# kai-neumann/OrthoSfM

Hardware: AMD Instinct MI355X
Metric: image-pairs matched/sec + BA iterations/sec (N images, M tracks) at 1/2/4/8 GPU (higher is better)
Workload: dtype i8; 1 GPU; 50 orthographic images, 20000 SIFT features/img, exhaustive matching (1225 pairs, low-res gate + two-way + cross-check + lists; SURVEY 8d's unit of work: up to, not including, RANSAC-F -- the pass through RANSAC-F is `with_geometric_verification`); views=50, features_per_view=20000, pairs=1225

## Files before the change

### orthosfm_amd/csrc/match_all.hip

```cpp
#include <algorithm>
#include <chrono>
#include <cstdlib>
#include <cstring>

#include "match_internal.h"
#include "ransac_kernels.h"
#include "ransac_affine.h"

namespace osfm {

namespace {

struct Lap {
    std::chrono::steady_clock::time_point t_chunk = std::chrono::steady_clock::now();
    void operator()(const char *what) const
    {
        static const bool trace = getenv("OSFM_MATCH_TRACE") != nullptr;
        if (trace) fprintf(stderr, "[osfm match] %-18s %9.3f ms\n", what,
            std::chrono::duration<double, std::milli>(std::chrono::steady_clock::now() - t_chunk).count());
    }
};

struct ChunkLists {
    std::vector<int64_t> m12_off, corr_off;
    std::vector<int32_t> len12;
    std::vector<uint8_t> keep;
};

int compact_chunk(osfm_matcher *m, const ChunkLists &h, int n, int64_t chunk_corr, int32_t *corr, int64_t written, int *chunk_no)
{
    const osfm_match_options &o = m->opts;
    hipStream_t s = m->stream;
    OSFM_RETURN_IF(m->d_m12_off.reserve(n * 8));
    OSFM_RETURN_IF(m->d_corr_off.reserve(n * 8));
    OSFM_RETURN_IF(m->d_len12.reserve(n * 4));
    OSFM_RETURN_IF(m->d_keep_pair.reserve(n));
    const int cb = o.geometric_verification ? 0 : ((*chunk_no)++ & 1);
    DeviceBuffer &dcorr = cb ? m->d_corr_alt : m->d_corr;
    if (m->copied_used[cb]) OSFM_HIP_CHECK(hipEventSynchronize(m->ev_copied[cb]));
    OSFM_RETURN_IF(dcorr.reserve((size_t)chunk_corr * 8));
    OSFM_HIP_CHECK(hipMemcpyAsync(m->d_m12_off.ptr, h.m12_off.data(), n * 8, hipMemcpyHostToDevice, s));
    OSFM_HIP_CHECK(hipMemcpyAsync(m->d_corr_off.ptr, h.corr_off.data(), n * 8, hipMemcpyHostToDevice, s));
    OSFM_HIP_CHECK(hipMemcpyAsync(m->d_len12.ptr, h.len12.data(), n * 4, hipMemcpyHostToDevice, s));
    OSFM_HIP_CHECK(hipMemcpyAsync(m->d_keep_pair.ptr, h.keep.data(), n, hipMemcpyHostToDevice, s));
    launch_compact_pairs(n, m->out.as<int32_t>(), m->d_m12_off.as<int64_t>(),
        m->d_len12.as<int32_t>(), m->d_corr_off.as<int64_t>(), m->d_keep_pair.as<uint8_t>(),
        dcorr.as<int32_t>(), s);
    OSFM_HIP_CHECK(hipGetLastError());
    if (!o.geometric_verification) {
        OSFM_HIP_CHECK(hipEventRecord(m->ev_compact[cb], s));
        OSFM_HIP_CHECK(hipStreamWaitEvent(m->copy_stream, m->ev_compact[cb], 0));
        OSFM_HIP_CHECK(hipMemcpyAsync(corr + 2 * written, dcorr.ptr, (size_t)chunk_corr * 8,
            hipMemcpyDeviceToHost, m->copy_stream));
        OSFM_HIP_CHECK(hipEventRecord(m->ev_copied[cb], m->copy_stream));
        m->copied_used[cb] = true;
    }
    return OSFM_OK;
}

int verify_chunk(osfm_matcher *m, const osfm_pair *pairs, const int *idx, int n, const std::vector<int32_t> &counts,
    const ChunkLists &h, int64_t chunk_corr, osfm_pair_result *results, int32_t *corr, int64_t capacity,
    int64_t *written_out, bool *overflow, const Lap &lap)
{
    const osfm_match_options &o = m->opts;
    hipStream_t s = m->stream;
    std::vector<RansacJob> jobs;
    std::vector<int> job_pair;
    OSFM_RETURN_IF(m->d_inl.reserve((size_t)chunk_corr * 4));
    OSFM_RETURN_IF(m->d_inl_count.reserve((size_t)n * 4));
    for (int k = 0; k < n; ++k) {
        if (!h.keep[k]) continue;
        const int p = idx[k];
        const ViewData &a = m->views[pairs[p].view_1], &b = m->views[pairs[p].view_2];
        if (a.n_positions < 0 || b.n_positions < 0) {
            set_error("match_all: geometric verification needs osfm_match_set_positions for views %d and %d",
                pairs[p].view_1, pairs[p].view_2);
            return OSFM_E_STATE;
        }
        RansacJob j;
        memset(&j, 0, sizeof(j));
        j.pos1 = a.positions.as<float>(); j.pos2 = b.positions.as<float>();
        j.corr = m->d_corr.as<int32_t>() + 2 * h.corr_off[k];
        j.k = counts[k];
        const int64_t hi = std::max(pairs[p].view_1, pairs[p].view_2), lo = std::min(pairs[p].view_1, pairs[p].view_2);
        j.pair_id = (uint64_t)(hi * (hi - 1) / 2 + lo);
        j.inliers_out = m->d_inl.as<int32_t>() + h.corr_off[k];
        j.count_out = m->d_inl_count.as<int32_t>() + (int)jobs.size();
        j.F_out = nullptr;
        jobs.push_back(j); job_pair.push_back(k);
    }
    const size_t jobs_bytes = (jobs.size() * sizeof(RansacJob) + 255) / 256 * 256;
    const bool affine = o.ransac_model == OSFM_RANSAC_AFFINE;
    OSFM_RETURN_IF(m->d_jobs.reserve(jobs_bytes + (affine ? affine_scratch_bytes((int)jobs.size()) : ransac_scratch_bytes((int)jobs.size()))));
    OSFM_HIP_CHECK(hipMemcpyAsync(m->d_jobs.ptr, jobs.data(), jobs.size() * sizeof(RansacJob), hipMemcpyHostToDevice, s));
    if (affine)
        launch_ransac_affine(m->d_jobs.as<RansacJob>(), (int)jobs.size(), o.ransac_max_iterations, o.ransac_threshold,
            o.ransac_refit, o.ransac_seed, static_cast<char *>(m->d_jobs.ptr) + jobs_bytes, nullptr, s);
    else
        launch_ransac(m->d_jobs.as<RansacJob>(), (int)jobs.size(), o.ransac_max_iterations, o.ransac_threshold,
            o.ransac_seed, static_cast<char *>(m->d_jobs.ptr) + jobs_bytes, s);
    OSFM_HIP_CHECK(hipGetLastError());
    std::vector<int32_t> h_cnt(jobs.size());
    OSFM_HIP_CHECK(hipMemcpyAsync(h_cnt.data(), m->d_inl_count.ptr, jobs.size() * 4, hipMemcpyDeviceToHost, s));
    lap("ransac queued");
    OSFM_HIP_CHECK(hipStreamSynchronize(s));
    lap("ransac done");
    const int min_inl = std::max(8, o.min_matching_inliers);
    std::vector<int64_t> g_src, g_dst;
    std::vector<int32_t> g_cnt;
    int64_t chunk_out = 0;
    for (size_t jx = 0; jx < jobs.size(); ++jx) {
        const int k = job_pair[jx];
        osfm_pair_result &r = results[idx[k]];
        r.num_inliers = h_cnt[jx];
        if (h_cnt[jx] < min_inl) { r.status = OSFM_PAIR_REJECTED_INLIERS; r.offset = 0; continue; }
        r.offset = *written_out + chunk_out;
        g_src.push_back(h.corr_off[k]); g_dst.push_back(chunk_out); g_cnt.push_back(h_cnt[jx]);
        chunk_out += h_cnt[jx];
    }
    if (*written_out + chunk_out > capacity) *overflow = true;
    if (!*overflow && chunk_out > 0) {
        const int ng = (int)g_cnt.size();
        OSFM_RETURN_IF(m->d_gather_off.reserve((size_t)ng * 20));
        OSFM_RETURN_IF(m->d_corr2.reserve((size_t)chunk_out * 8));
        char *gb = m->d_gather_off.as<char>();
        OSFM_HIP_CHECK(hipMemcpyAsync(gb, g_src.data(), (size_t)ng * 8, hipMemcpyHostToDevice, s));
        OSFM_HIP_CHECK(hipMemcpyAsync(gb + (size_t)ng * 8, g_dst.data(), (size_t)ng * 8, hipMemcpyHostToDevice, s));
        OSFM_HIP_CHECK(hipMemcpyAsync(gb + (size_t)ng * 16, g_cnt.data(), (size_t)ng * 4, hipMemcpyHostToDevice, s));
        launch_gather_inliers(ng, m->d_corr.as<int32_t>(), m->d_inl.as<int32_t>(),
            reinterpret_cast<const int64_t *>(gb), reinterpret_cast<const int64_t *>(gb + (size_t)ng * 8),
            reinterpret_cast<const int32_t *>(gb + (size_t)ng * 16), m->d_corr2.as<int32_t>(), s);
        OSFM_HIP_CHECK(hipGetLastError());
        OSFM_HIP_CHECK(hipMemcpyAsync(corr + 2 * *written_out, m->d_corr2.ptr, (size_t)chunk_out * 8,
            hipMemcpyDeviceToHost, s));
        OSFM_HIP_CHECK(hipStreamSynchronize(s));
        lap("lists on the host");
    }
    *written_out += chunk_out;
    return OSFM_OK;
}

}

int match_all_single(osfm_matcher *m, const osfm_pair *pairs, int num_pairs, osfm_pair_result *results,
    int32_t *corr, int64_t capacity, int64_t *total, int phase)
{
    std::lock_guard<std::mutex> lock(m->mu);
    OSFM_HIP_CHECK(hipSetDevice(m->device));
    if (phase != kPhaseFull) reset_stats(m);
    const osfm_match_options &o = m->opts;
    struct CopyDrain { hipStream_t s; ~CopyDrain() { if (s) (void)hipStreamSynchronize(s); } } copy_drain{m->copy_stream};

    std::vector<int> lowres_idx, full_idx;
    for (int p = 0; p < num_pairs; ++p) {
        OSFM_RETURN_IF(check_view(m, pairs[p].view_1, "match_all"));
        OSFM_RETURN_IF(check_view(m, pairs[p].view_2, "match_all"));
        const ViewData &a = m->views[pairs[p].view_1], &b = m->views[pairs[p].view_2];
        osfm_pair_result &r = results[p];
        if (phase == kPhaseFull) {
            if (r.status == OSFM_PAIR_MATCHED) full_idx.push_back(p);
            continue;
        }
        r.status = OSFM_PAIR_MATCHED; r.lowres_matches = -1; r.num_matches = 0; r.num_inliers = -1; r.offset = 0;
        const size_t np1 = (size_t)a.ns + a.nu, np2 = (size_t)b.ns + b.nu;
        if (np1 == 0 || np2 == 0) { r.status = OSFM_PAIR_SKIPPED_EMPTY; continue; }
        if (o.use_lowres_matching && np1 * np2 > 1000000) lowres_idx.push_back(p);
        else full_idx.push_back(p);
    }

    {
        const int bs = batch_size_for(m->views, o, true);
        std::vector<osfm_pair> chunk;
        for (size_t start = 0; start < lowres_idx.size(); start += bs) {
            const size_t end = std::min(lowres_idx.size(), start + bs);
            chunk.clear();
            for (size_t k = start; k < end; ++k) chunk.push_back(pairs[lowres_idx[k]]);
            BatchResult res;
            BatchMode mode;
            mode.limit = o.num_lowres_features; mode.lowres = true; mode.apply = false;
            OSFM_RETURN_IF(run_batch(m, chunk.data(), (int)chunk.size(), mode, &res));
            for (size_t k = start; k < end; ++k) {
                const int p = lowres_idx[k];
                results[p].lowres_matches = res.counts[k - start];
                if (res.counts[k - start] < o.min_lowres_matches)
                    results[p].status = OSFM_PAIR_REJECTED_LOWRES;
                else
                    full_idx.push_back(p);
            }
        }
        std::sort(full_idx.begin(), full_idx.end());
    }
    if (phase == kPhaseGate) { if (total) *total = 0; return OSFM_OK; }

    const int min_matches = std::max(8, o.min_feature_matches);
    int64_t written = 0, written_out = 0;
    bool overflow = false;
    {
        const int bs = full_batch_size(m->views, o, full_idx.size());
        int chunk_no = 0;
        std::vector<osfm_pair> chunk;
        ChunkLists h;
        for (size_t start = 0; start < full_idx.size(); start += bs) {
            const size_t end = std::min(full_idx.size(), start + bs);
            const int n = (int)(end - start);
            chunk.clear();
            for (size_t k = start; k < end; ++k) chunk.push_back(pairs[full_idx[k]]);
            const Lap lap{};
            BatchResult res;
            BatchMode full_mode;
            if (m->expect_pairs > 0)
                full_mode.expect = std::min<int>(full_batch_size(m->views, o, (size_t)m->expect_pairs), m->expect_pairs);
            OSFM_RETURN_IF(run_batch(m, chunk.data(), n, full_mode, &res));
            lap("matched");
            h.m12_off.assign(n, 0); h.corr_off.assign(n, 0); h.len12.assign(n, 0); h.keep.assign(n, 0);
            int64_t chunk_corr = 0;
            for (int k = 0; k < n; ++k) {
                const int p = full_idx[start + k];
                osfm_pair_result &r = results[p];
                r.num_matches = res.counts[k];
                if (res.counts[k] < min_matches) { r.status = OSFM_PAIR_REJECTED_COUNT; continue; }
                r.status = OSFM_PAIR_MATCHED;
                r.offset = written + chunk_corr;
                h.keep[k] = 1;
                h.m12_off[k] = res.plans[k].off12;
                h.len12[k] = res.plans[k].len12;
                h.corr_off[k] = chunk_corr;
                chunk_corr += res.counts[k];
            }
            if (!o.geometric_verification && written + chunk_corr > capacity) overflow = true;
            if (chunk_corr > 0 && (o.geometric_verification || !overflow))
                OSFM_RETURN_IF(compact_chunk(m, h, n, chunk_corr, corr, written, &chunk_no));
            if (o.geometric_verification && chunk_corr > 0)
                OSFM_RETURN_IF(verify_chunk(m, pairs, full_idx.data() + start, n, res.counts, h, chunk_corr, results, corr,
                    capacity, &written_out, &overflow, lap));
            written += chunk_corr;
        }
    }
    if (!o.geometric_verification) OSFM_HIP_CHECK(hipStreamSynchronize(m->copy_stream));
    if (o.geometric_verification) written = written_out;
    if (total) *total = written;
    if (overflow) {
        set_error("match_all: %lld correspondences need more than the given capacity %lld",
            (long long)written, (long long)capacity);
        return OSFM_E_CAPACITY;
    }
    return OSFM_OK;
}

}
```

### orthosfm_amd/csrc/match_api.hip

```cpp
#include <algorithm>
#include <cfloat>
#include <cmath>
#include <cstddef>
#include <cstring>

#include "match_internal.h"
#include "cashash_kernels.h"
#include "ransac_kernels.h"
#include "ransac_affine.h"
#include "view_front.h"

namespace osfm {

static thread_local std::string g_last_error;

void set_error(const char *fmt, ...)
{
    char buf[1024];
    va_list ap;
    va_start(ap, fmt);
    vsnprintf(buf, sizeof(buf), fmt, ap);
    va_end(ap);
    g_last_error = buf;
}

}

using namespace osfm;

extern "C" {

const char *osfm_last_error(void) { return g_last_error.c_str(); }
int osfm_version(void) { return OSFM_ABI_VERSION; }

int osfm_device_count(void)
{
    int n = 0;
    if (hipGetDeviceCount(&n) != hipSuccess) return 0;
    return n;
}

int osfm_ransac_selfcheck(int mode, uint64_t *counters)
{
    if (mode < 0 || mode > 2) { set_error("ransac_selfcheck: mode %d", mode); return OSFM_E_ARG; }
    int ndev = 0;
    if (hipGetDeviceCount(&ndev) != hipSuccess || ndev <= 0) {
        set_error("ransac_selfcheck: no HIP device available");
        return OSFM_E_DEVICE;
    }
    unsigned long long c[3] = {0, 0, 0};
    OSFM_RETURN_IF(ransac_set_mode(mode, c));
    if (counters) for (int i = 0; i < 3; ++i) counters[i] = c[i];
    return OSFM_OK;
}

int osfm_trim_device_memory(int device, uint64_t *released_bytes)
{
    int ndev = 0;
    if (hipGetDeviceCount(&ndev) != hipSuccess || ndev <= 0) {
        set_error("trim_device_memory: no HIP device available");
        return OSFM_E_DEVICE;
    }
    if (device < -1 || device >= ndev) { set_error("trim_device_memory: device %d out of range [-1,%d)", device, ndev); return OSFM_E_ARG; }
    const size_t b = g_device_pool.trim(device);
    if (released_bytes) *released_bytes = b;
    return OSFM_OK;
}

int osfm_device_memory(int device, uint64_t *free_bytes, uint64_t *total_bytes)
{
    int ndev = 0;
    if (hipGetDeviceCount(&ndev) != hipSuccess || ndev <= 0) {
        set_error("device_memory: no HIP device available");
        return OSFM_E_DEVICE;
    }
    if (device < 0 || device >= ndev) { set_error("device_memory: device %d out of range [0,%d)", device, ndev); return OSFM_E_ARG; }
    OSFM_HIP_CHECK(hipSetDevice(device));
    size_t f = 0, t = 0;
    OSFM_HIP_CHECK(hipMemGetInfo(&f, &t));
    if (free_bytes) *free_bytes = f;
    if (total_bytes) *total_bytes = t;
    return OSFM_OK;
}

int osfm_library_memory(osfm_memory_report *out)
{
    if (!out) { set_error("library_memory: null"); return OSFM_E_ARG; }
    out->device_buffer_bytes = g_ledger.device_buffer_bytes.load();
    out->pool_live_bytes = g_ledger.pool_live_bytes.load();
    out->pool_cached_bytes = g_ledger.pool_cached_bytes.load();
    out->pinned_host_bytes = g_ledger.pinned_host_bytes.load();
    out->live_matchers = g_ledger.live_matchers.load();
    out->live_streams = g_ledger.live_streams.load();
    out->live_events = g_ledger.live_events.load();
    out->reserved = 0;
    return OSFM_OK;
}

int osfm_match_options_default(osfm_match_options *o)
{
    if (!o) { set_error("options_default: null"); return OSFM_E_ARG; }
    o->sift_lowe_ratio = 0.8f;
    o->sift_distance_threshold = FLT_MAX;
    o->surf_lowe_ratio = 0.7f;
    o->surf_distance_threshold = FLT_MAX;
    o->use_lowres_matching = 1;
    o->num_lowres_features = 500;
    o->min_lowres_matches = 5;
    o->min_feature_matches = 50;
    o->pairs_per_batch = 0;
    o->geometric_verification = 0;
    o->ransac_max_iterations = 1000;
    o->ransac_threshold = 0.0015;
    o->min_matching_inliers = 30;
    o->matcher_type = OSFM_MATCHER_EXHAUSTIVE;
    o->ransac_seed = 0;
    o->cascade_keep_empty_blocks = 0;
    o->special_kernel_max = 0;
    o->ransac_model = OSFM_RANSAC_FUNDAMENTAL;
    o->ransac_refit = 1;
    return OSFM_OK;
}

int osfm_match_create(int device, int num_views, const osfm_match_options *opts, osfm_matcher **out)
{
    if (!out || num_views < 0) { set_error("match_create: bad arguments"); return OSFM_E_ARG; }
    *out = nullptr;
    if (opts && opts->ransac_model != OSFM_RANSAC_FUNDAMENTAL && opts->ransac_model != OSFM_RANSAC_AFFINE) {
        set_error("match_create: ransac_model %d", opts->ransac_model);
        return OSFM_E_ARG;
    }
    int ndev = 0;
    if (hipGetDeviceCount(&ndev) != hipSuccess || ndev <= 0) {
        set_error("match_create: no HIP device available (this backend has no CPU fallback)");
        return OSFM_E_DEVICE;
    }
    if (device < 0 || device >= ndev) {
        set_error("match_create: device %d out of range [0,%d)", device, ndev);
        return OSFM_E_ARG;
    }
    OSFM_HIP_CHECK(hipSetDevice(device));
    struct Owner { osfm_matcher *p; ~Owner() { if (p) osfm_match_destroy(p); } } owner{(g_ledger.live_matchers++, new osfm_matcher())};
    osfm_matcher *m = owner.p;
    m->device = device;
    if (opts) m->opts = *opts; else osfm_match_options_default(&m->opts);
    m->views = std::vector<ViewData>(num_views);
    reset_stats(m);
    OSFM_HIP_CHECK(stream_create(&m->stream));
    for (int i = 0; i < 2; ++i)
        for (int j = 0; j < 2; ++j) OSFM_HIP_CHECK(event_create(&m->ev[i][j], true));
    for (int j = 0; j < 2; ++j) OSFM_HIP_CHECK(event_create(&m->ev_sp[j], true));
    for (int j = 0; j < 2; ++j) OSFM_HIP_CHECK(event_create(&m->pin_ev[j], false));
    OSFM_HIP_CHECK(stream_create(&m->copy_stream));
    OSFM_HIP_CHECK(stream_create(&m->up_stream));
    for (int j = 0; j < 2; ++j) {
        OSFM_HIP_CHECK(event_create(&m->ev_compact[j], false));
        OSFM_HIP_CHECK(event_create(&m->ev_copied[j], false));
    }
    if (m->opts.special_kernel_max != 0) m->special_max = std::min(std::max(m->opts.special_kernel_max, 0), 512);
    std::vector<int32_t> t;
    build_lowe_table(m->opts.sift_lowe_ratio, false, &t);
    OSFM_RETURN_IF(m->lowe_sift.reserve(t.size() * 4));
    OSFM_HIP_CHECK(hipMemcpy(m->lowe_sift.ptr, t.data(), t.size() * 4, hipMemcpyHostToDevice));
    build_lowe_table(m->opts.surf_lowe_ratio, true, &t);
    OSFM_RETURN_IF(m->lowe_surf.reserve(t.size() * 4));
    OSFM_HIP_CHECK(hipMemcpy(m->lowe_surf.ptr, t.data(), t.size() * 4, hipMemcpyHostToDevice));
    m->tab_sift.reject_from = m->lowe_sift.as<int32_t>();
    m->tab_sift.max_d1 = max_d1_for(m->opts.sift_distance_threshold, false);
    m->tab_sift.is_signed = 0;
    m->tab_surf.reject_from = m->lowe_surf.as<int32_t>();
    m->tab_surf.max_d1 = max_d1_for(m->opts.surf_distance_threshold, true);
    m->tab_surf.is_signed = 1;
    owner.p = nullptr;
    *out = m;
    return OSFM_OK;
}

int osfm_match_create_multi(const int *device_ids, int num_devices, int num_views,
    const osfm_match_options *opts, osfm_matcher **out)
{
    if (!out || !device_ids || num_devices < 1 || num_views < 0) { set_error("match_create_multi: bad arguments"); return OSFM_E_ARG; }
    *out = nullptr;
    if (opts && opts->ransac_model != OSFM_RANSAC_FUNDAMENTAL && opts->ransac_model != OSFM_RANSAC_AFFINE) {
        set_error("match_create_multi: ransac_model %d", opts->ransac_model);
        return OSFM_E_ARG;
    }
    struct Owner { osfm_matcher *p; ~Owner() { if (p) osfm_match_destroy(p); } } owner{(g_ledger.live_matchers++, new osfm_matcher())};
    osfm_matcher *m = owner.p;
    m->device = device_ids[0];
    if (opts) m->opts = *opts; else osfm_match_options_default(&m->opts);
    reset_stats(m);
    for (int k = 0; k < num_devices; ++k) {
        osfm_matcher *sh = nullptr;
        OSFM_RETURN_IF(osfm_match_create(device_ids[k], num_views, &m->opts, &sh));
        m->shards.push_back(sh);
    }
    m->shard_stage.resize(num_devices);
    owner.p = nullptr;
    *out = m;
    return OSFM_OK;
}

int osfm_match_get_devices(const osfm_matcher *m, int32_t *device_ids, int capacity, int32_t *num_devices)
{
    if (!m || !num_devices || capacity < 0 || (capacity > 0 && !device_ids)) { set_error("match_get_devices: bad arguments"); return OSFM_E_ARG; }
    const int n = m->shards.empty() ? 1 : (int)m->shards.size();
    *num_devices = n;
    for (int k = 0; k < std::min(n, capacity); ++k) device_ids[k] = m->shards.empty() ? m->device : m->shards[k]->device;
    return OSFM_OK;
}

int osfm_match_destroy(osfm_matcher *m)
{
    if (!m) return OSFM_OK;
    if (!m->shards.empty() || !m->shard_stage.empty()) {
        for (auto *sh : m->shards) osfm_match_destroy(sh);
        for (auto &sg : m->shard_stage) pinned_free(sg.ptr, sg.ints * 4);
        g_ledger.live_matchers--;
        delete m;
        return OSFM_OK;
    }
    (void)hipSetDevice(m->device);
    if (m->stream) (void)hipStreamSynchronize(m->stream);
    for (int i = 0; i < 2; ++i)
        for (int j = 0; j < 2; ++j) event_destroy(m->ev[i][j]);
    for (int j = 0; j < 2; ++j) event_destroy(m->ev_sp[j]);
    for (int j = 0; j < 2; ++j) {
        event_destroy(m->pin_ev[j]);
        pinned_free(m->pin_ptr[j], m->pin_bytes[j]);
    }
    stream_destroy(m->copy_stream);
    stream_destroy(m->up_stream);
    for (int j = 0; j < 2; ++j) {
        event_destroy(m->ev_compact[j]);
        event_destroy(m->ev_copied[j]);
    }
    stream_destroy(m->stream);
    for (auto *sg : m->comb_staging) { pinned_free(sg->ptr, sg->ints * 4); delete sg; }
    g_ledger.live_matchers--;
    delete m;
    return OSFM_OK;
}

int osfm_quantize_sift(const float *src, int n, uint16_t *dst)
{
    if (n < 0 || (n > 0 && (!src || !dst))) { set_error("quantize_sift: bad arguments"); return OSFM_E_ARG; }
    for (size_t i = 0; i < (size_t)n * 128; ++i) {
        float v = src[i];
        v = v < 0.0f ? 0.0f : (v > 1.0f ? 1.0f : v);
        v *= 255.0f;
        v = v > 0.0f ? floorf(v + 0.5f) : ceilf(v - 0.5f);
        dst[i] = (uint16_t)(unsigned char)v;
    }
    return OSFM_OK;
}

int osfm_quantize_surf(const float *src, int n, int16_t *dst)
{
    if (n < 0 || (n > 0 && (!src || !dst))) { set_error("quantize_surf: bad arguments"); return OSFM_E_ARG; }
    for (size_t i = 0; i < (size_t)n * 64; ++i) {
        float v = src[i];
        v = v < -1.0f ? -1.0f : (v > 1.0f ? 1.0f : v);
        v *= 127.0f;
        v = v > 0.0f ? floorf(v + 0.5f) : ceilf(v - 0.5f);
        dst[i] = (int16_t)(signed char)v;
    }
    return OSFM_OK;
}

int osfm_match_set_view(osfm_matcher *m, int view, const uint16_t *sift, int n_sift,
    const int16_t *surf, int n_surf)
{
    if (!m) { set_error("set_view: null matcher"); return OSFM_E_ARG; }
    if (!m->shards.empty())
        return for_each_shard(m, [&](size_t k) { return osfm_match_set_view(m->shards[k], view, sift, n_sift, surf, n_surf); });
    std::lock_guard<std::mutex> lock(m->up_mu);
    OSFM_HIP_CHECK(hipSetDevice(m->device));
    return upload_view(m, view, sift, n_sift, surf, n_surf);
}

int osfm_match_set_view_float(osfm_matcher *m, int view, const float *sift, int n_sift,
    const float *surf, int n_surf)
{
    if (!m) { set_error("set_view_float: null matcher"); return OSFM_E_ARG; }
    if (n_sift < 0 || n_surf < 0) { set_error("set_view_float: negative count"); return OSFM_E_ARG; }
    std::vector<uint16_t> qs((size_t)n_sift * 128);
    std::vector<int16_t> qu((size_t)n_surf * 64);
    OSFM_RETURN_IF(osfm_quantize_sift(sift, n_sift, qs.data()));
    OSFM_RETURN_IF(osfm_quantize_surf(surf, n_surf, qu.data()));
    return osfm_match_set_view(m, view, qs.data(), n_sift, qu.data(), n_surf);
}

int osfm_match_expect_pairs(osfm_matcher *m, int32_t pairs_per_call)
{
    if (!m || pairs_per_call < 0) { set_error("match_expect_pairs: bad arguments"); return OSFM_E_ARG; }
    if (!m->shards.empty()) {
        for (auto *sh : m->shards) sh->expect_pairs = (pairs_per_call + (int)m->shards.size() - 1) / (int)m->shards.size();
        return OSFM_OK;
    }
    std::lock_guard<std::mutex> lock(m->mu);
    m->expect_pairs = pairs_per_call;
    return OSFM_OK;
}

int osfm_match_view_size(const osfm_matcher *m, int view, int *n_sift, int *n_surf)
{
    if (!m) { set_error("view_size: null matcher"); return OSFM_E_ARG; }
    if (!m->shards.empty()) return osfm_match_view_size(m->shards[0], view, n_sift, n_surf);
    OSFM_RETURN_IF(check_view(m, view, "view_size"));
    if (n_sift) *n_sift = m->views[view].ns;
    if (n_surf) *n_surf = m->views[view].nu;
    return OSFM_OK;
}

int osfm_match_set_positions(osfm_matcher *m, int view, const float *xy, int n)
{
    if (!m || n < 0 || (n > 0 && !xy)) { set_error("set_positions: bad argument"); return OSFM_E_ARG; }
    if (!m->shards.empty())
        return for_each_shard(m, [&](size_t k) { return osfm_match_set_positions(m->shards[k], view, xy, n); });
    std::lock_guard<std::mutex> lock(m->mu);
    OSFM_HIP_CHECK(hipSetDevice(m->device));
    OSFM_RETURN_IF(check_view(m, view, "set_positions"));
    ViewData &v = m->views[view];
    if (n != v.ns + v.nu) {
        set_error("set_positions: view %d has %d features, got %d positions", view, v.ns + v.nu, n);
        return OSFM_E_ARG;
    }
    OSFM_RETURN_IF(v.positions.reserve((size_t)std::max(n, 1) * 8));
    if (n) OSFM_HIP_CHECK(hipMemcpy(v.positions.ptr, xy, (size_t)n * 8, hipMemcpyHostToDevice));
    v.n_positions = n;
    return OSFM_OK;
}

int osfm_match_set_view_from_front(osfm_matcher *m, int view, osfm_view_front *front)
{
    if (!m || !front) { set_error("set_view_from_front: null argument"); return OSFM_E_ARG; }
    FrontResult r;
    OSFM_RETURN_IF(view_front_result(front, &r));
    return handoff_all(m, view, r.device, r.sift_desc, r.sift_map, r.n_sift, r.surf_desc, r.surf_map, r.n_surf, r.normalized,
        [&](hipStream_t s) { return view_front_begin_read(front, s); }, [&](hipStream_t s) { return view_front_end_read(front, s); });
}

int osfm_match_debug_set_view_device(osfm_matcher *m, int view, const float *sift, int n_sift, const int32_t *sift_order,
    const float *surf, int n_surf, const int32_t *surf_order, const float *positions)
{
    if (!m || n_sift < 0 || n_surf < 0 || (n_sift > 0 && !sift) || (n_surf > 0 && !surf) || (n_sift + n_surf > 0 && !positions)) {
        set_error("debug_set_view_device: bad arguments");
        return OSFM_E_ARG;
    }
    for (int i = 0; i < n_sift; ++i)
        if (sift_order && (sift_order[i] < 0 || sift_order[i] >= n_sift)) { set_error("debug_set_view_device: sift_order[%d] out of range", i); return OSFM_E_ARG; }
    for (int i = 0; i < n_surf; ++i)
        if (surf_order && (surf_order[i] < 0 || surf_order[i] >= n_surf)) { set_error("debug_set_view_device: surf_order[%d] out of range", i); return OSFM_E_ARG; }
    const int device = m->shards.empty() ? m->device : m->shards[0]->device;
    OSFM_HIP_CHECK(hipSetDevice(device));
    DeviceBuffer d_sift, d_surf, d_so, d_uo, d_pos;
    auto put = [](DeviceBuffer &b, const void *src, size_t bytes) -> int {
        if (!src || !bytes) return OSFM_OK;
        OSFM_RETURN_IF(b.reserve(bytes));
        OSFM_HIP_CHECK(hipMemcpy(b.ptr, src, bytes, hipMemcpyHostToDevice));
        return OSFM_OK;
    };
    OSFM_RETURN_IF(put(d_sift, sift, (size_t)n_sift * 128 * 4));
    OSFM_RETURN_IF(put(d_surf, surf, (size_t)n_surf * 64 * 4));
    OSFM_RETURN_IF(put(d_so, sift_order, (size_t)n_sift * 4));
    OSFM_RETURN_IF(put(d_uo, surf_order, (size_t)n_surf * 4));
    OSFM_RETURN_IF(put(d_pos, positions, (size_t)(n_sift + n_surf) * 8));
    hipStream_t used = nullptr;
    const int rc = handoff_all(m, view, device, d_sift.as<float>(), d_so.as<int32_t>(), n_sift, d_surf.as<float>(), d_uo.as<int32_t>(),
        n_surf, d_pos.as<float>(), [&](hipStream_t s) -> int { used = s; return OSFM_OK; }, [](hipStream_t) -> int { return OSFM_OK; });
    if (used) (void)hipStreamSynchronize(used);
    return rc;
}

int osfm_match_debug_view_bank(osfm_matcher *m, int view, int shard, osfm_view_bank *b)
{
    if (!m || !b) { set_error("debug_view_bank: null argument"); return OSFM_E_ARG; }
    if (!m->shards.empty()) {
        if (shard < 0 || shard >= (int)m->shards.size()) { set_error("debug_view_bank: shard %d of %zu", shard, m->shards.size()); return OSFM_E_ARG; }
        return osfm_match_debug_view_bank(m->shards[(size_t)shard], view, 0, b);
    }
    std::lock_guard<std::mutex> lock(m->up_mu);
    OSFM_HIP_CHECK(hipSetDevice(m->device));
    OSFM_RETURN_IF(check_view(m, view, "debug_view_bank"));
    const ViewData &v = m->views[view];
    OSFM_HIP_CHECK(hipStreamSynchronize(m->up_stream));
    const int sp_pad = v.n_special > 0 ? round_up(v.n_special, kRowsPerBlock) : 0;
    b->n_sift = v.ns; b->n_surf = v.nu; b->n_sift_pad = v.ns_pad; b->n_surf_pad = v.nu_pad;
    b->n_special = v.n_special; b->n_special_pad = sp_pad; b->surf_norm2_max = v.surf_norm2_max; b->n_positions = v.n_positions;
    struct { void *to; const DeviceBuffer *from; size_t bytes; } arrays[] = {
        {b->sift, &v.sift, (size_t)v.ns_pad * 128}, {b->sift_corr, &v.sift_corr, (size_t)v.ns_pad * 4},
        {b->sift_raw, &v.sift_raw, (size_t)v.ns_pad * 128}, {b->sift_raw_corr, &v.sift_raw_corr, (size_t)v.ns_pad * 4},
        {b->surf, &v.surf, (size_t)v.nu_pad * 64}, {b->surf_corr, &v.surf_corr, (size_t)v.nu_pad * 4},
        {b->special, &v.special, (size_t)sp_pad * 128}, {b->special_corr, &v.special_corr, (size_t)sp_pad * 4},
        {b->special_map, &v.special_map, sp_pad ? (size_t)v.n_special * 4 : 0},
        {b->special_slot, &v.special_slot, sp_pad ? (size_t)v.ns * 4 : 0},
        {b->positions, &v.positions, (size_t)std::max(v.n_positions, 0) * 8},
    };
    for (auto &r : arrays)
        if (r.to && r.bytes) OSFM_HIP_CHECK(hipMemcpy(r.to, r.from->ptr, r.bytes, hipMemcpyDeviceToHost));
    return OSFM_OK;
}

int osfm_ransac_options_default(osfm_ransac_options *o)
{
    if (!o) { set_error("ransac_options_default: null"); return OSFM_E_ARG; }
    o->max_iterations = 1000; o->reserved = 0; o->threshold = 0.0015; o->seed = 0;
    return OSFM_OK;
}

}

template <class Launch>
static int ransac_single_pair(const char *name, int min_k, size_t scratch_bytes, int device, const float *pos1, int n1,
    const float *pos2, int n2, const int32_t *corr, int k, uint64_t pair_id, int32_t *inliers, int32_t *num_inliers,
    double *F, void *result, size_t result_bytes, Launch launch)
{
    if (n1 < 0 || n2 < 0 || k < 0 || !num_inliers || (k > 0 && (!pos1 || !pos2 || !corr || !inliers))) {
        set_error("%s: bad argument", name); return OSFM_E_ARG;
    }
    for (int i = 0; i < k; ++i)
        if (corr[2 * i] < 0 || corr[2 * i] >= n1 || corr[2 * i + 1] < 0 || corr[2 * i + 1] >= n2) {
            set_error("%s: correspondence %d out of range", name, i); return OSFM_E_ARG;
        }
    int ndev = 0;
    if (hipGetDeviceCount(&ndev) != hipSuccess || ndev <= 0) {
        set_error("%s: no HIP device available (this backend has no CPU fallback)", name);
        return OSFM_E_DEVICE;
    }
    if (device < 0 || device >= ndev) { set_error("%s: bad device", name); return OSFM_E_ARG; }
    OSFM_HIP_CHECK(hipSetDevice(device));
    if (k < min_k) { *num_inliers = -1; return OSFM_OK; }
    DeviceBuffer d1, d2, dc, di, dn, df, dj, dr;
    struct Rel { DeviceBuffer *b[8]; ~Rel() { for (auto *x : b) x->release(); } } rel{{&d1, &d2, &dc, &di, &dn, &df, &dj, &dr}};
    OSFM_RETURN_IF(d1.reserve((size_t)n1 * 8)); OSFM_RETURN_IF(d2.reserve((size_t)n2 * 8));
    OSFM_RETURN_IF(dc.reserve((size_t)k * 8)); OSFM_RETURN_IF(di.reserve((size_t)k * 4));
    OSFM_RETURN_IF(dn.reserve(16)); OSFM_RETURN_IF(df.reserve(72));
    if (result_bytes) OSFM_RETURN_IF(dr.reserve(result_bytes));
    OSFM_RETURN_IF(dj.reserve(256 + scratch_bytes));
    OSFM_HIP_CHECK(hipMemcpy(d1.ptr, pos1, (size_t)n1 * 8, hipMemcpyHostToDevice));
    OSFM_HIP_CHECK(hipMemcpy(d2.ptr, pos2, (size_t)n2 * 8, hipMemcpyHostToDevice));
    OSFM_HIP_CHECK(hipMemcpy(dc.ptr, corr, (size_t)k * 8, hipMemcpyHostToDevice));
    RansacJob job;
    memset(&job, 0, sizeof(job));
    job.pos1 = d1.as<float>(); job.pos2 = d2.as<float>(); job.corr = dc.as<int32_t>(); job.k = k;
    job.pair_id = pair_id; job.inliers_out = di.as<int32_t>(); job.count_out = dn.as<int32_t>();
    job.F_out = df.as<double>();
    OSFM_HIP_CHECK(hipMemcpy(dj.ptr, &job, sizeof(job), hipMemcpyHostToDevice));
    launch(dj.as<RansacJob>(), static_cast<char *>(dj.ptr) + 256, dr.ptr);
    OSFM_HIP_CHECK(hipGetLastError());
    OSFM_HIP_CHECK(hipDeviceSynchronize());
    int32_t cnt = 0;
    OSFM_HIP_CHECK(hipMemcpy(&cnt, dn.ptr, 4, hipMemcpyDeviceToHost));
    *num_inliers = cnt;
    if (cnt > 0) OSFM_HIP_CHECK(hipMemcpy(inliers, di.ptr, (size_t)cnt * 4, hipMemcpyDeviceToHost));
    if (F) OSFM_HIP_CHECK(hipMemcpy(F, df.ptr, 72, hipMemcpyDeviceToHost));
    if (result) OSFM_HIP_CHECK(hipMemcpy(result, dr.ptr, result_bytes, hipMemcpyDeviceToHost));
    return OSFM_OK;
}

extern "C" {

int osfm_ransac_fundamental(int device, const float *pos1, int n1, const float *pos2, int n2,
    const int32_t *corr, int k, const osfm_ransac_options *opts, uint64_t pair_id,
    int32_t *inliers, int32_t *num_inliers, double *F)
{
    osfm_ransac_options o;
    if (opts) o = *opts; else osfm_ransac_options_default(&o);
    return ransac_single_pair("ransac_fundamental", 8, ransac_scratch_bytes(1), device, pos1, n1, pos2, n2, corr, k, pair_id,
        inliers, num_inliers, F, nullptr, 0, [&](const RansacJob *d_job, void *scratch, void *) {
            launch_ransac(d_job, 1, o.max_iterations, o.threshold, o.seed, scratch, nullptr);
        });
}

int osfm_ransac_affine_options_default(osfm_ransac_affine_options *o)
{
    if (!o) { set_error("ransac_affine_options_default: null"); return OSFM_E_ARG; }
    o->max_iterations = 1000; o->refit = 1; o->threshold = 0.0015; o->seed = 0;
    return OSFM_OK;
}

int osfm_ransac_affine(int device, const float *pos1, int n1, const float *pos2, int n2,
    const int32_t *corr, int k, const osfm_ransac_affine_options *opts, uint64_t pair_id,
    int32_t *inliers, int32_t *num_inliers, double *F, osfm_ransac_affine_result *result)
{
    osfm_ransac_affine_options o;
    if (opts) o = *opts; else osfm_ransac_affine_options_default(&o);
    return ransac_single_pair("ransac_affine", 4, affine_scratch_bytes(1), device, pos1, n1, pos2, n2, corr, k, pair_id,
        inliers, num_inliers, F, result, sizeof(*result), [&](const RansacJob *d_job, void *scratch, void *d_result) {
            launch_ransac_affine(d_job, 1, o.max_iterations, o.threshold, o.refit, o.seed, scratch,
                static_cast<osfm_ransac_affine_result *>(d_result), nullptr);
        });
}

int osfm_match_pair(osfm_matcher *m, int view_1, int view_2, int32_t *m12, int32_t *len12,
    int32_t *m21, int32_t *len21)
{
    if (!m || !m12 || !m21) { set_error("match_pair: null argument"); return OSFM_E_ARG; }
    if (!m->shards.empty())
        return osfm_match_pair(m->shards[m->next_shard++ % m->shards.size()], view_1, view_2, m12, len12, m21, len21);
    OSFM_RETURN_IF(check_view(m, view_1, "match"));
    OSFM_RETURN_IF(check_view(m, view_2, "match"));
    osfm_matcher::PairRequest rq;
    rq.kind = 0; rq.v1 = view_1; rq.v2 = view_2; rq.num_features = 0;
    rq.m12 = m12; rq.m21 = m21; rq.len12 = len12; rq.len21 = len21; rq.count = nullptr;
    return combine(m, rq);
}

int osfm_match_pair_lowres(osfm_matcher *m, int view_1, int view_2, int num_features, int32_t *count)
{
    if (!m || !count) { set_error("match_pair_lowres: null argument"); return OSFM_E_ARG; }
    if (!m->shards.empty())
        return osfm_match_pair_lowres(m->shards[m->next_shard++ % m->shards.size()], view_1, view_2, num_features, count);
    if (num_features <= 0) { *count = 0; return OSFM_OK; }
    OSFM_RETURN_IF(check_view(m, view_1, "match"));
    OSFM_RETURN_IF(check_view(m, view_2, "match"));
    osfm_matcher::PairRequest rq;
    rq.kind = 1; rq.v1 = view_1; rq.v2 = view_2; rq.num_features = num_features;
    rq.m12 = rq.m21 = rq.len12 = rq.len21 = nullptr; rq.count = count;
    return combine(m, rq);
}

int osfm_match_twoway(osfm_matcher *m, int view_1, int view_2, int descriptor_type, int num_features,
    int32_t *m12, int32_t *m21)
{
    if (!m || !m12 || !m21 || (descriptor_type != 0 && descriptor_type != 1) || num_features < 0) {
        set_error("match_twoway: bad argument");
        return OSFM_E_ARG;
    }
    if (!m->shards.empty()) return osfm_match_twoway(m->shards[0], view_1, view_2, descriptor_type, num_features, m12, m21);
    std::lock_guard<std::mutex> lock(m->mu);
    OSFM_HIP_CHECK(hipSetDevice(m->device));
    reset_stats(m);
    osfm_pair pr = {view_1, view_2};
    BatchResult res;
    BatchMode mode;
    mode.limit = num_features; mode.apply = false; mode.type_mask = 1 << descriptor_type;
    OSFM_RETURN_IF(run_batch(m, &pr, 1, mode, &res));
    const PairPlan &pl = res.plans[0];
    const ViewData &a = m->views[view_1], &b = m->views[view_2];
    int n1 = descriptor_type == 0 ? a.ns : a.nu, n2 = descriptor_type == 0 ? b.ns : b.nu;
    if (num_features > 0) { n1 = std::min(n1, num_features); n2 = std::min(n2, num_features); }
    if (n1 == 0) { for (int i = 0; i < n2; ++i) m21[i] = -1; return OSFM_OK; }
    const int32_t *d_out = m->out.as<int32_t>();
    if (pl.len12) OSFM_HIP_CHECK(hipMemcpy(m12, d_out + pl.off12, (size_t)pl.len12 * 4, hipMemcpyDeviceToHost));
    if (pl.len21) OSFM_HIP_CHECK(hipMemcpy(m21, d_out + pl.off21, (size_t)pl.len21 * 4, hipMemcpyDeviceToHost));
    return OSFM_OK;
}

int osfm_pair_from_index(int64_t index, int32_t *view_1, int32_t *view_2)
{
    if (index < 0 || !view_1 || !view_2) { set_error("pair_from_index: bad arguments"); return OSFM_E_ARG; }
    const int a = (int)(0.5 + std::sqrt(0.25 + 2.0 * (double)index));
    *view_1 = a;
    *view_2 = (int)index - a * (a - 1) / 2;
    return OSFM_OK;
}

int osfm_match_all(osfm_matcher *m, const osfm_pair *pairs, int num_pairs, osfm_pair_result *results,
    int32_t *corr, int64_t capacity, int64_t *total)
{
    if (!m || (num_pairs > 0 && (!pairs || !results)) || num_pairs < 0 || capacity < 0 ||
        (capacity > 0 && !corr)) {
        set_error("match_all: bad arguments");
        return OSFM_E_ARG;
    }
    if (!m->shards.empty()) return multi_match_all(m, pairs, num_pairs, results, corr, capacity, total);
    return match_all_single(m, pairs, num_pairs, results, corr, capacity, total, kPhaseBoth);
}

int osfm_match_get_cascade_hashes(osfm_matcher *m, int view, int type, uint64_t *hashes,
    uint8_t *bucket_ids)
{
    if (!m || type < 0 || type > 1) { set_error("get_cascade_hashes: bad arguments"); return OSFM_E_ARG; }
    if (!m->shards.empty()) return osfm_match_get_cascade_hashes(m->shards[0], view, type, hashes, bucket_ids);
    std::lock_guard<std::mutex> lock(m->mu);
    OSFM_RETURN_IF(check_view(m, view, "get_cascade_hashes"));
    OSFM_HIP_CHECK(hipSetDevice(m->device));
    OSFM_RETURN_IF(ensure_cashash(m));
    const ViewData &v = m->views[view];
    const int n = type == 0 ? v.ns : v.nu;
    const int words = type == 0 ? 2 : 1;
    if (n > 0 && hashes)
        OSFM_HIP_CHECK(hipMemcpy(hashes, v.cas_hash[type].ptr, (size_t)n * words * 8, hipMemcpyDeviceToHost));
    if (n > 0 && bucket_ids)
        OSFM_HIP_CHECK(hipMemcpy(bucket_ids, v.cas_bucket[type].ptr, (size_t)n * kCasGroups, hipMemcpyDeviceToHost));
    return OSFM_OK;
}

int osfm_match_get_shard_stats(const osfm_matcher *m, int shard, osfm_match_stats *out)
{
    if (!m || !out) { set_error("get_shard_stats: null argument"); return OSFM_E_ARG; }
    const int n = m->shards.empty() ? 1 : (int)m->shards.size();
    if (shard < 0 || shard >= n) { set_error("get_shard_stats: shard %d of %d", shard, n); return OSFM_E_ARG; }
    *out = m->shards.empty() ? m->stats : m->shards[shard]->stats;
    return OSFM_OK;
}

int osfm_match_get_stats(const osfm_matcher *m, osfm_match_stats *out)
{
    if (!m || !out) { set_error("get_stats: null argument"); return OSFM_E_ARG; }
    if (!m->shards.empty()) {
        memset(out, 0, sizeof(*out));
        for (const auto *sh : m->shards) {
            const osfm_match_stats &t = sh->stats;
            out->tile_kernel_ms += t.tile_kernel_ms; out->tile_kernel_launches += t.tile_kernel_launches;
            out->exact_scan_queries += t.exact_scan_queries; out->mac_count += t.mac_count;
            out->algorithmic_bytes += t.algorithmic_bytes; out->lowres_kernel_ms += t.lowres_kernel_ms;
            out->lowres_kernel_launches += t.lowres_kernel_launches; out->lowres_mac_count += t.lowres_mac_count;
            out->cashash_kernel_ms += t.cashash_kernel_ms; out->cashash_kernel_launches += t.cashash_kernel_launches;
            out->special_kernel_launches += t.special_kernel_launches; out->special_kernel_ms += t.special_kernel_ms;
            out->tile_shader_cycles += t.tile_shader_cycles; out->tile_refclk_ticks += t.tile_refclk_ticks;
            out->surf_tile_kernel_ms += t.surf_tile_kernel_ms; out->surf_tile_kernel_launches += t.surf_tile_kernel_launches;
            out->surf_mac_count += t.surf_mac_count; out->tile_workgroups += t.tile_workgroups;
        }
        return OSFM_OK;
    }
    *out = m->stats;
    return OSFM_OK;
}

#undef osfm_match_options_default
#undef osfm_match_create
#undef osfm_match_create_multi
static constexpr size_t kOptionsBytesBefore = offsetof(osfm_match_options, ransac_model);
static_assert(kOptionsBytesBefore == 80, "the layout binaries built against the earlier header pass");

static osfm_match_options options_from_before(const void *opts)
{
    osfm_match_options o;
    memset(&o, 0, sizeof(o));
    osfm_match_options_default_v2(&o);
    if (opts) memcpy(&o, opts, kOptionsBytesBefore);
    return o;
}

OSFM_API int osfm_match_options_default(void *opts)
{
    if (!opts) { set_error("options_default: null"); return OSFM_E_ARG; }
    const osfm_match_options o = options_from_before(nullptr);
    memcpy(opts, &o, kOptionsBytesBefore);
    return OSFM_OK;
}

OSFM_API int osfm_match_create(int device, int num_views, const void *opts, osfm_matcher **out)
{
    const osfm_match_options o = options_from_before(opts);
    return osfm_match_create_v2(device, num_views, &o, out);
}

OSFM_API int osfm_match_create_multi(const int *device_ids, int num_devices, int num_views, const void *opts, osfm_matcher **out)
{
    const osfm_match_options o = options_from_before(opts);
    return osfm_match_create_multi_v2(device_ids, num_devices, num_views, &o, out);
}

}
```

### orthosfm_amd/csrc/match_batch.hip

```cpp
#include <algorithm>
#include <cstdlib>
#include <cstring>

#include "match_internal.h"
#include "cashash_kernels.h"

namespace osfm {

int check_view(const osfm_matcher *m, int v, const char *what) { return check_view(m->views, v, what); }

void reset_stats(osfm_matcher *m) { memset(&m->stats, 0, sizeof(m->stats)); }

int run_batch(osfm_matcher *m, const osfm_pair *pairs, int num_pairs, const BatchMode &mode,
    BatchResult *res)
{
    const bool cascade = cascade_batch(m->opts, mode);
    if (cascade) OSFM_RETURN_IF(ensure_cashash(m));
    static const int forced_seg_tiles = [] { const char *e = getenv("OSFM_SEG_TILES"); return e ? atoi(e) : 0; }();
    const char *rescan_env = getenv("OSFM_FINISH_RESCAN");
    PlanKnobs knobs;
    knobs.seg_tiles = forced_seg_tiles;
    knobs.rescan_wave = rescan_env && strcmp(rescan_env, "wave") == 0;
    BatchPlan &plan = m->plan;
    res->counts.assign(num_pairs, 0);
    OSFM_RETURN_IF(plan_batch(m->views, m->opts, m->special_max, knobs, pairs, num_pairs, mode, &plan));
    res->plans = plan.plans;
    res->out_ints = plan.out_ints;
    const std::vector<PairPlan> &plans = plan.plans;
    std::vector<MatchProblem> *probs = plan.probs;
    const std::vector<SpecialJob> &spjobs = plan.spjobs, &spjobs_wide = plan.spjobs_wide;
    const int64_t out_ints = plan.out_ints, total_queries = plan.total_queries, rs_buckets = plan.rs_buckets;
    const int *total_blocks = plan.total_blocks, *max_n = plan.max_n;

    double grow = 1.0;
    if (mode.expect > num_pairs && num_pairs > 0) grow = 1.02 * (double)mode.expect / num_pairs;
    auto grown = [&](int64_t n) { return (size_t)((double)std::max<int64_t>(n, 1) * std::max(grow, 1.0)); };
    OSFM_RETURN_IF(m->out.reserve(grown(std::max<int64_t>(out_ints, 4)) * 4));
    OSFM_RETURN_IF(m->rowparts.reserve(grown(plan.rowpart_recs) * sizeof(RowPart)));
    OSFM_RETURN_IF(m->colparts.reserve(grown(plan.colpart_recs) * sizeof(ColPart)));
    OSFM_RETURN_IF(m->keep.reserve(grown(std::max<int64_t>(plan.keep_bytes, 16))));
    OSFM_RETURN_IF(m->exact_items.reserve(grown(total_queries) * sizeof(ExactItem)));
    OSFM_RETURN_IF(m->exact_count.reserve(16));
    if (plan.bucketed) {
        OSFM_RETURN_IF(m->rs_count.reserve(grown(rs_buckets) * sizeof(int32_t)));
        OSFM_RETURN_IF(m->rs_items.reserve(grown(plan.rs_items) * sizeof(RescoreItem)));
    }
    OSFM_RETURN_IF(m->sp_parts.reserve((size_t)std::max<int64_t>(plan.sp_recs, 1) * sizeof(RowPart)));
    hipStream_t s = m->stream;
    {
        std::vector<uint8_t> seen(m->views.size(), 0);
        for (int p = 0; p < num_pairs; ++p)
            for (int v : {plans[p].v1, plans[p].v2})
                if (!seen[v]) { seen[v] = 1; if (m->views[v].ready) OSFM_HIP_CHECK(hipStreamWaitEvent(s, m->views[v].ready, 0)); }
    }
    OSFM_RETURN_IF(m->sp_col.reserve((size_t)std::max<int64_t>(plan.sp_cols, 1) * 4));
    OSFM_RETURN_IF(m->d_spjobs.reserve(std::max<size_t>(spjobs.size() + spjobs_wide.size(), 1) * sizeof(SpecialJob)));
    if (!spjobs.empty())
        OSFM_HIP_CHECK(hipMemcpyAsync(m->d_spjobs.ptr, spjobs.data(), spjobs.size() * sizeof(SpecialJob),
            hipMemcpyHostToDevice, s));
    if (!spjobs_wide.empty())
        OSFM_HIP_CHECK(hipMemcpyAsync(m->d_spjobs.as<SpecialJob>() + spjobs.size(), spjobs_wide.data(),
            spjobs_wide.size() * sizeof(SpecialJob), hipMemcpyHostToDevice, s));
    int32_t *d_out = m->out.as<int32_t>();
    OSFM_HIP_CHECK(hipMemsetAsync(d_out, 0xff, (size_t)std::max<int64_t>(out_ints, 4) * 4, s));

    OSFM_HIP_CHECK(hipMemsetAsync(m->exact_count.ptr, 0, 16, s));
    bool timed[2] = {false, false};
    bool probed = false;
    for (int type = 0; type < 2; ++type) {
        const int np = (int)probs[type].size();
        if (np == 0) continue;
        for (int i = 0; i < np; ++i) {
            probs[type][i].m12 = d_out + plan.m12_off[type][i];
            probs[type][i].m21 = d_out + plan.m21_off[type][i];
        }
        OSFM_RETURN_IF(m->d_problems[type].reserve(np * sizeof(MatchProblem)));
        OSFM_RETURN_IF(m->mark_off[type].reserve(np * 2 * sizeof(int64_t)));
        OSFM_RETURN_IF(m->counts[type].reserve(np * sizeof(int32_t)));
        OSFM_HIP_CHECK(hipMemcpyAsync(m->d_problems[type].ptr, probs[type].data(),
            np * sizeof(MatchProblem), hipMemcpyHostToDevice, s));
        OSFM_HIP_CHECK(hipMemcpyAsync(m->mark_off[type].ptr, plan.mark_off[type].data(),
            np * 2 * sizeof(int64_t), hipMemcpyHostToDevice, s));
        OSFM_HIP_CHECK(hipMemsetAsync(m->counts[type].ptr, 0, np * sizeof(int32_t), s));
        const MatchProblem *dp = m->d_problems[type].as<MatchProblem>();
        const LoweTable tab = type == 0 ? m->tab_sift : m->tab_surf;
        const int ecap = (int)std::min<int64_t>(total_queries, 0x7fffffff);
        int32_t *ecount = m->exact_count.as<int32_t>() + type;

        if (cascade) {
            OSFM_HIP_CHECK(hipEventRecord(m->ev[type][0], s));
            timed[type] = true;
            OSFM_RETURN_IF(m->cas_state.reserve((size_t)std::max<int64_t>(plan.cas_queries[type], 1) * kCasMaxCand * 4));
            launch_cashash_match(type == 0 ? 128 : 64, dp, np, max_n[type], m->cas_state.as<int32_t>(), tab, s);
            OSFM_HIP_CHECK(hipEventRecord(m->ev[type][1], s));
        } else {
            if (total_blocks[type] > 0) { OSFM_HIP_CHECK(hipEventRecord(m->ev[type][0], s)); timed[type] = true; }
            unsigned long long *probe = nullptr;
            if (type == 0 && mode.limit == 0) {
                OSFM_RETURN_IF(m->clock_probe.reserve(16));
                OSFM_HIP_CHECK(hipMemsetAsync(m->clock_probe.ptr, 0, 16, s));
                probe = m->clock_probe.as<unsigned long long>();
                probed = true;
            }
            if (!m->zero_tile.ptr) {
                OSFM_RETURN_IF(m->zero_tile.reserve((size_t)kTileCols * 128));
                OSFM_HIP_CHECK(hipMemsetAsync(m->zero_tile.ptr, 0, (size_t)kTileCols * 128, s));
            }
            launch_match_tiles(type == 0 ? 8 : 4, plan.needs_mask[type], plan.any_special[type], plan.any_c0[type],
                plan.any_corrected[type], dp, np, total_blocks[type],
                m->rowparts.as<RowPart>(), m->colparts.as<ColPart>(), s, probe, m->zero_tile.as<int8_t>());
            if (timed[type]) OSFM_HIP_CHECK(hipEventRecord(m->ev[type][1], s));
            if (type == 0 && !(spjobs.empty() && spjobs_wide.empty())) {
                OSFM_HIP_CHECK(hipEventRecord(m->ev_sp[0], s));
                launch_match_special(dp, m->d_spjobs.as<SpecialJob>(), (int)spjobs.size(), m->sp_parts.as<RowPart>(),
                    m->sp_col.as<int32_t>(), s);
                launch_match_special_wide(dp, m->d_spjobs.as<SpecialJob>() + spjobs.size(), (int)spjobs_wide.size(),
                    m->sp_parts.as<RowPart>(), m->sp_col.as<int32_t>(), s);
                OSFM_HIP_CHECK(hipEventRecord(m->ev_sp[1], s));
            }
            const bool rs = type == 0 && plan.bucketed;
            if (rs) OSFM_HIP_CHECK(hipMemsetAsync(m->rs_count.ptr, 0, (size_t)rs_buckets * sizeof(int32_t), s));
            launch_match_finish(dp, np, max_n[type], m->rowparts.as<RowPart>(),
                m->colparts.as<ColPart>(), m->sp_parts.as<RowPart>(), m->sp_col.as<int32_t>(), tab, 0,
                m->exact_items.as<ExactItem>(), ecount, ecap, rs ? m->rs_count.as<int32_t>() : nullptr,
                rs ? m->rs_items.as<RescoreItem>() : nullptr, s);
            if (rs)
                launch_match_rescore(dp, np, m->rs_count.as<int32_t>(), m->rs_items.as<RescoreItem>(), rs_buckets, tab,
                    m->exact_items.as<ExactItem>(), ecount, ecap, s);
            launch_exact_scan(type == 0 ? 128 : 64, dp, m->exact_items.as<ExactItem>(), ecount, ecap,
                tab, s);
        }
        launch_cross_check_mark(dp, np, max_n[type], m->keep.as<uint8_t>(), m->keep.as<uint8_t>(),
            m->mark_off[type].as<int64_t>(), m->counts[type].as<int32_t>(), s);
        if (mode.apply)
            launch_cross_check_apply(dp, np, max_n[type], m->keep.as<uint8_t>(),
                m->keep.as<uint8_t>(), m->mark_off[type].as<int64_t>(), s);
        OSFM_HIP_CHECK(hipGetLastError());
    }

    std::vector<int32_t> hc[2];
    int32_t hexact[4] = {0, 0, 0, 0};
    for (int type = 0; type < 2; ++type) {
        hc[type].resize(probs[type].size());
        if (!hc[type].empty())
            OSFM_HIP_CHECK(hipMemcpyAsync(hc[type].data(), m->counts[type].ptr,
                hc[type].size() * sizeof(int32_t), hipMemcpyDeviceToHost, s));
    }
    OSFM_HIP_CHECK(hipMemcpyAsync(hexact, m->exact_count.ptr, 16, hipMemcpyDeviceToHost, s));
    unsigned long long hprobe[2] = {0, 0};
    if (probed) OSFM_HIP_CHECK(hipMemcpyAsync(hprobe, m->clock_probe.ptr, 16, hipMemcpyDeviceToHost, s));
    OSFM_HIP_CHECK(hipStreamSynchronize(s));
    m->stats.tile_shader_cycles += (double)hprobe[0];
    m->stats.tile_refclk_ticks += (double)hprobe[1];
    for (int p = 0; p < num_pairs; ++p) {
        int c = 0;
        for (int type = 0; type < 2; ++type)
            if (plans[p].prob_index[type] >= 0) c += hc[type][plans[p].prob_index[type]];
        res->counts[p] = c;
    }
    for (int type = 0; type < 2; ++type) {
        if (!timed[type]) continue;
        float ms = 0.f;
        OSFM_HIP_CHECK(hipEventElapsedTime(&ms, m->ev[type][0], m->ev[type][1]));
        if (cascade) {
            m->stats.cashash_kernel_ms += ms;
            m->stats.cashash_kernel_launches += 1;
        } else if (mode.limit > 0) {
            m->stats.lowres_kernel_ms += ms;
            m->stats.lowres_kernel_launches += 1;
        } else {
            m->stats.tile_kernel_ms += ms;
            m->stats.tile_kernel_launches += 1;
            m->stats.tile_workgroups += total_blocks[type];
            if (type == 1) { m->stats.surf_tile_kernel_ms += ms; m->stats.surf_tile_kernel_launches += 1; }
        }
    }
    if (!(spjobs.empty() && spjobs_wide.empty())) {
        float ms = 0.f;
        OSFM_HIP_CHECK(hipEventElapsedTime(&ms, m->ev_sp[0], m->ev_sp[1]));
        m->stats.special_kernel_ms += ms;
        m->stats.special_kernel_launches += 1;
    }
    m->stats.exact_scan_queries += hexact[0] + hexact[1];
    if (cascade) {
    } else if (mode.limit > 0) {
        m->stats.lowres_mac_count += plan.macs;
    } else {
        m->stats.mac_count += plan.macs;
        m->stats.surf_mac_count += plan.macs_surf;
        m->stats.algorithmic_bytes += plan.alg_bytes;
    }
    return OSFM_OK;
}

}
```

### orthosfm_amd/csrc/match_internal.h

```cpp
#pragma once
#include <atomic>
#include <condition_variable>
#include <deque>
#include <functional>
#include <mutex>
#include <string>
#include <vector>

#include "match_plan.h"

struct osfm_matcher {
    int device = 0;
    hipStream_t stream = nullptr;
    osfm_match_options opts;
    std::vector<osfm::ViewData> views;
    osfm::DeviceBuffer lowe_sift, lowe_surf;
    osfm::LoweTable tab_sift, tab_surf;
    std::mutex mu;
    hipStream_t up_stream = nullptr;
    std::mutex up_mu;

    osfm::DeviceBuffer d_problems[2], rowparts, colparts, out, keep, mark_off[2], counts[2];
    osfm::DeviceBuffer exact_items, exact_count, stage_in, flags;
    osfm::DeviceBuffer rs_count, rs_items;
    osfm::DeviceBuffer sp_parts, sp_col, d_spjobs;
    osfm::DeviceBuffer clock_probe;
    osfm::BatchPlan plan;
    osfm::DeviceBuffer zero_tile;
    int special_max = 512;
    int expect_pairs = 0;
    osfm::DeviceBuffer d_m12_off, d_len12, d_corr_off, d_keep_pair, d_corr;
    osfm::DeviceBuffer d_corr_alt;
    hipStream_t copy_stream = nullptr;
    hipEvent_t ev_compact[2] = {nullptr, nullptr}, ev_copied[2] = {nullptr, nullptr};
    bool copied_used[2] = {false, false};
    osfm::DeviceBuffer d_jobs, d_inl, d_inl_count, d_corr2, d_gather_off;
    hipEvent_t ev[2][2] = {{nullptr, nullptr}, {nullptr, nullptr}};
    hipEvent_t ev_sp[2] = {nullptr, nullptr};
    char *pin_ptr[2] = {nullptr, nullptr};
    size_t pin_bytes[2] = {0, 0};
    hipEvent_t pin_ev[2] = {nullptr, nullptr};
    bool pin_used[2] = {false, false};
    unsigned pin_next = 0;

    osfm::DeviceBuffer cas_proj[2], cas_sum[2], cas_avg[2], cas_state;
    std::atomic<bool> cas_dirty{true};

    osfm_match_stats stats;

    struct Staging { int32_t *ptr = nullptr; size_t ints = 0; int users = 0; };
    struct PairRequest {
        int kind;
        int v1, v2, num_features;
        int32_t *m12, *m21, *len12, *len21, *count;
        int status = OSFM_OK;
        bool done = false;
        std::string error;
        Staging *stage = nullptr;
        int64_t src12 = 0, src21 = 0;
        int32_t n12 = 0, n21 = 0;
    };
    std::vector<Staging *> comb_staging;

    std::vector<osfm_matcher *> shards;
    std::vector<Staging> shard_stage;
    std::atomic<unsigned> next_shard{0};
    std::mutex multi_mu;
    std::mutex comb_mu;
    std::condition_variable comb_cv;
    std::deque<PairRequest *> comb_queue;
    bool comb_leader = false;
};

namespace osfm {

int check_view(const osfm_matcher *m, int v, const char *what);
int run_batch(osfm_matcher *m, const osfm_pair *pairs, int num_pairs, const BatchMode &mode, BatchResult *res);
void reset_stats(osfm_matcher *m);

int upload_view(osfm_matcher *m, int view, const uint16_t *sift, int n_sift, const int16_t *surf, int n_surf);
int handoff_all(osfm_matcher *m, int view, int device, const float *d_sift, const int32_t *sift_map, int n_sift,
    const float *d_surf, const int32_t *surf_map, int n_surf, const float *d_positions,
    const std::function<int(hipStream_t)> &begin, const std::function<int(hipStream_t)> &end);
int ensure_cashash(osfm_matcher *m);

enum { kPhaseBoth = 0, kPhaseGate = 1, kPhaseFull = 2 };
int match_all_single(osfm_matcher *m, const osfm_pair *pairs, int num_pairs, osfm_pair_result *results,
    int32_t *corr, int64_t capacity, int64_t *total, int phase);

int for_each_shard(osfm_matcher *m, const std::function<int(size_t)> &fn);
int multi_match_all(osfm_matcher *m, const osfm_pair *pairs, int num_pairs, osfm_pair_result *results,
    int32_t *corr, int64_t capacity, int64_t *total);

int combine(osfm_matcher *m, osfm_matcher::PairRequest &rq);

}
```

### orthosfm_amd/csrc/match_plan.h

```cpp
#pragma once
#include <cstdint>
#include <vector>

#include "match_kernels.h"
#include "osfm_common.h"

namespace osfm {

inline int round_up(int x, int m) { return (x + m - 1) / m * m; }

struct ViewData {
    bool set = false;
    int ns = 0, nu = 0;
    int ns_pad = 0, nu_pad = 0;
    DeviceBuffer sift, sift_corr, surf, surf_corr;
    DeviceBuffer sift_raw, sift_raw_corr, special, special_corr, special_map, special_slot;
    int n_special = 0;
    int surf_norm2_max = 0;
    DeviceBuffer cas_hash[2], cas_bucket[2], cas_start[2], cas_items[2], cas_rec[2];
    DeviceBuffer positions;
    int n_positions = -1;
    hipEvent_t ready = nullptr;
    ~ViewData() { event_destroy(ready); }
    ViewData() = default;
    ViewData(const ViewData &) = delete;
    ViewData &operator=(const ViewData &) = delete;
};

struct PairPlan {
    int v1, v2;
    int ns1, nu1, ns2, nu2;
    bool has_sift, has_surf;
    int64_t off12, off21;
    int len12, len21;
    int prob_index[2];
};

struct BatchResult {
    std::vector<PairPlan> plans;
    std::vector<int32_t> counts;
    int64_t out_ints = 0;
};

struct BatchMode {
    int limit = 0;
    bool lowres = false;
    bool apply = true;
    int type_mask = 3;
    int expect = 0;
};

inline bool cascade_batch(const osfm_match_options &opts, const BatchMode &mode)
{
    return opts.matcher_type == OSFM_MATCHER_CASCADE_HASHING && mode.limit == 0;
}

struct PlanKnobs {
    int seg_tiles = 0;
    bool rescan_wave = false;
};

struct BatchPlan {
    std::vector<PairPlan> plans;
    std::vector<MatchProblem> probs[2];
    std::vector<int64_t> m12_off[2], m21_off[2];
    std::vector<int64_t> mark_off[2];
    std::vector<SpecialJob> spjobs, spjobs_wide;
    int64_t out_ints = 0, rowpart_recs = 0, colpart_recs = 0, keep_bytes = 0, total_queries = 0;
    int64_t sp_recs = 0, sp_cols = 0;
    int64_t rs_buckets = 0, rs_items = 0;
    int64_t cas_queries[2] = {0, 0};
    int total_blocks[2] = {0, 0}, max_n[2] = {0, 0};
    bool needs_mask[2] = {false, false};
    bool any_special[2] = {false, false};
    bool any_c0[2] = {false, false}, any_corrected[2] = {false, false};
    bool bucketed = false, cascade = false;
    int64_t macs = 0, macs_surf = 0, alg_bytes = 0;
    void clear();
};

int check_view(const std::vector<ViewData> &views, int v, const char *what);

int plan_batch(const std::vector<ViewData> &views, const osfm_match_options &opts, int special_max, const PlanKnobs &knobs,
    const osfm_pair *pairs, int num_pairs, const BatchMode &mode, BatchPlan *out);

int batch_size_for(const std::vector<ViewData> &views, const osfm_match_options &o, bool lowres);
int full_batch_size(const std::vector<ViewData> &views, const osfm_match_options &o, size_t n_full);

void deal_pairs_lpt(const std::vector<ViewData> &views, int num_shards, const osfm_pair *pairs, const std::vector<int> &cand,
    std::vector<std::vector<int>> *owner);

void build_lowe_table(float lowe, bool is_signed, std::vector<int32_t> *tab);
int max_d1_for(float dist_thres, bool is_signed);

}
```

### orthosfm_amd/csrc/match_plan.hip

```cpp
#include <algorithm>
#include <climits>
#include <cstring>
#include <queue>

#include "match_plan.h"

namespace osfm {

int check_view(const std::vector<ViewData> &views, int v, const char *what)
{
    if (v < 0 || v >= (int)views.size()) {
        set_error("%s: view id %d out of range [0, %zu)", what, v, views.size());
        return OSFM_E_ARG;
    }
    if (!views[v].set) {
        set_error("%s: view %d has not been set", what, v);
        return OSFM_E_STATE;
    }
    return OSFM_OK;
}

void BatchPlan::clear()
{
    BatchPlan fresh;
    auto keep = [](auto &to, auto &from) { from.clear(); to.swap(from); };
    keep(fresh.plans, plans);
    keep(fresh.spjobs, spjobs);
    keep(fresh.spjobs_wide, spjobs_wide);
    for (int type = 0; type < 2; ++type) {
        keep(fresh.probs[type], probs[type]);
        keep(fresh.m12_off[type], m12_off[type]);
        keep(fresh.m21_off[type], m21_off[type]);
        keep(fresh.mark_off[type], mark_off[type]);
    }
    *this = std::move(fresh);
}

int plan_batch(const std::vector<ViewData> &views, const osfm_match_options &opts, int special_max, const PlanKnobs &knobs,
    const osfm_pair *pairs, int num_pairs, const BatchMode &mode, BatchPlan *out)
{
    BatchPlan &bp = *out;
    bp.clear();
    const int lowres_limit = mode.limit;
    const bool cascade = bp.cascade = cascade_batch(opts, mode);
    bp.plans.assign(num_pairs, PairPlan());
    struct SpEntry { int problem, side, view, units, nchunk; };
    std::vector<SpEntry> spentries;

    int64_t rb_estimate = 0;
    for (int p = 0; p < num_pairs; ++p) {
        const int v1 = pairs[p].view_1;
        if (v1 >= 0 && v1 < (int)views.size())
            rb_estimate += (std::max(views[v1].ns, views[v1].nu) + kRowsPerBlock - 1) / kRowsPerBlock;
    }
    auto choose_seg_cols = [&](int n2) {
        const int ncyc = (n2 + kCycleCols - 1) / kCycleCols;
        int cyc;
        if (knobs.seg_tiles > 0) cyc = std::max(1, knobs.seg_tiles / 16);
        else {
            constexpr int64_t kWantBlocks = 2048;
            const int64_t want = (kWantBlocks + std::max<int64_t>(rb_estimate, 1) - 1) / std::max<int64_t>(rb_estimate, 1);
            const int nseg = (int)std::min<int64_t>(std::max<int64_t>(want, 1), ncyc);
            cyc = (ncyc + nseg - 1) / nseg;
        }
        cyc = std::min(cyc, kSegColsMax / kCycleCols);
        return cyc * kCycleCols;
    };

    for (int p = 0; p < num_pairs; ++p) {
        PairPlan &pl = bp.plans[p];
        pl.v1 = pairs[p].view_1; pl.v2 = pairs[p].view_2;
        OSFM_RETURN_IF(check_view(views, pl.v1, "match"));
        OSFM_RETURN_IF(check_view(views, pl.v2, "match"));
        const ViewData &a = views[pl.v1], &b = views[pl.v2];
        pl.ns1 = a.ns; pl.nu1 = a.nu; pl.ns2 = b.ns; pl.nu2 = b.nu;
        pl.has_sift = a.ns > 0 && (mode.type_mask & 1);
        pl.has_surf = a.nu > 0 && (mode.type_mask & 2);
        if (cascade && !opts.cascade_keep_empty_blocks) {
            if (b.ns == 0) pl.has_sift = false;
            if (b.nu == 0) pl.has_surf = false;
        }
        if (mode.lowres && pl.has_sift) pl.has_surf = false;
        if (lowres_limit > 0) {
            pl.ns1 = std::min(pl.ns1, lowres_limit); pl.ns2 = std::min(pl.ns2, lowres_limit);
            pl.nu1 = std::min(pl.nu1, lowres_limit); pl.nu2 = std::min(pl.nu2, lowres_limit);
        }
        const int e1 = pl.has_sift ? pl.ns1 : 0;
        const int e2 = pl.has_sift ? pl.ns2 : 0;
        pl.len12 = e1 + (pl.has_surf ? pl.nu1 : 0);
        pl.len21 = e2 + (pl.has_surf ? pl.nu2 : 0);
        pl.off12 = bp.out_ints; bp.out_ints += round_up(pl.len12, 4);
        pl.off21 = bp.out_ints; bp.out_ints += round_up(pl.len21, 4);
        pl.prob_index[0] = pl.prob_index[1] = -1;
        for (int type = 0; type < 2; ++type) {
            if (type == 0 ? !pl.has_sift : !pl.has_surf) continue;
            MatchProblem pr;
            memset(&pr, 0, sizeof(pr));
            pr.n1 = type == 0 ? pl.ns1 : pl.nu1;
            pr.n2 = type == 0 ? pl.ns2 : pl.nu2;
            pr.A = (type == 0 ? a.sift : a.surf).as<int8_t>();
            pr.B = (type == 0 ? b.sift : b.surf).as<int8_t>();
            pr.corrA = (type == 0 ? a.sift_corr : a.surf_corr).as<int32_t>();
            pr.corrB = (type == 0 ? b.sift_corr : b.surf_corr).as<int32_t>();
            pr.A_raw = (type == 0 ? a.sift_raw : a.surf).as<int8_t>();
            pr.corrA_raw = (type == 0 ? a.sift_raw_corr : a.surf_corr).as<int32_t>();
            const bool limited = lowres_limit > 0;
            const int n_special = (type == 0 && !limited) ? a.n_special : 0;
            pr.n_special = n_special;
            pr.A_special = a.special.as<int8_t>();
            pr.corrA_special = a.special_corr.as<int32_t>();
            pr.special_map = a.special_map.as<int32_t>();
            pr.special_slot = n_special > 0 ? a.special_slot.as<int32_t>() : nullptr;
            const bool empty = pr.n1 == 0 || pr.n2 == 0;
            if (limited) bp.needs_mask[type] = true;
            pr.B_raw = (type == 0 ? b.sift_raw : b.surf).as<int8_t>();
            pr.c0 = (type == 1 || b.n_special == 0) ? 1 : 0;
            if (type == 0 && !limited && !cascade && !empty && (a.n_special > 0 || b.n_special > 0) &&
                a.n_special <= special_max && b.n_special <= special_max) {
                pr.sp = 1; pr.c0 = 1;
                pr.nsA = a.n_special; pr.nsB = b.n_special;
                pr.n_special = 0;
                pr.special_slot = a.n_special > 0 ? a.special_slot.as<int32_t>() : nullptr;
                pr.B_special = b.special.as<int8_t>();
                pr.corrB_special = b.special_corr.as<int32_t>();
                pr.special_map_B = b.special_map.as<int32_t>();
                pr.special_slot_B = b.n_special > 0 ? b.special_slot.as<int32_t>() : nullptr;
                for (int side = 0; side < 2; ++side) {
                    const int ns = side == 0 ? pr.nsA : pr.nsB, no = side == 0 ? pr.n2 : pr.n1;
                    if (ns == 0) continue;
                    const int units = (ns + 31) / 32;
                    pr.sp_wide[side] = units > kSpSlots ? 1 : 0;
                    const int chunk_cols = pr.sp_wide[side] ? kSpWideChunk : kSpChunk;
                    const int nchunk = (no + chunk_cols - 1) / chunk_cols;
                    pr.sp_row_off[side] = bp.sp_recs; bp.sp_recs += (int64_t)nchunk * round_up(ns, 32);
                    pr.sp_col_off[side] = bp.sp_cols; bp.sp_cols += round_up(no, 32);
                    spentries.push_back({(int)bp.probs[type].size(), side, side == 0 ? pl.v2 : pl.v1, units, nchunk});
                }
            }
            if (!empty && !limited) (pr.c0 ? bp.any_c0 : bp.any_corrected)[type] = true;
            if (!empty && pr.n_special > 0) bp.any_special[type] = true;
            pr.nrb_main = empty ? 0 : (pr.n1 + kRowsPerBlock - 1) / kRowsPerBlock;
            pr.nrb = pr.nrb_main + (empty ? 0 : (pr.n_special + kRowsPerBlock - 1) / kRowsPerBlock);
            pr.seg_cols = (pr.c0 && !limited && pr.n_special == 0 && !empty) ? choose_seg_cols(pr.n2) : kSegCols;
            pr.nseg = empty ? 0 : (pr.n2 + pr.seg_cols - 1) / pr.seg_cols;
            pr.n2stride = round_up(pr.n2, kCycleCols);
            pr.block_start = bp.total_blocks[type];
            pr.rs_bucket_off = bp.rs_buckets;
            pr.rs_item_off = bp.rs_items;
            if (type == 0 && !cascade && !empty) {
                bp.rs_buckets += rescore_buckets(pr.nrb_main, pr.n2);
                bp.rs_items += rescore_items(pr.nrb_main, pr.n2);
            }
            if (cascade) {
                const ViewData *vd[2] = {&a, &b};
                for (int side = 0; side < 2; ++side) {
                    pr.cas_rec[side] = vd[side]->cas_rec[type].ptr;
                    pr.cas_start[side] = vd[side]->cas_start[type].as<int32_t>();
                    pr.cas_items[side] = vd[side]->cas_items[type].as<int32_t>();
                }
                pr.cas_state_off[0] = bp.cas_queries[type]; bp.cas_queries[type] += pr.n1;
                pr.cas_state_off[1] = bp.cas_queries[type]; bp.cas_queries[type] += pr.n2;
            } else {
                bp.total_blocks[type] += pr.nrb * pr.nseg;
                pr.rowpart_off = bp.rowpart_recs;
                bp.rowpart_recs += (int64_t)pr.nseg * pr.nrb * kRowsPerBlock;
                pr.colpart_off = bp.colpart_recs;
                bp.colpart_recs += (int64_t)pr.nrb * pr.n2stride;
            }
            bp.m12_off[type].push_back(pl.off12 + (type == 0 ? 0 : e1));
            bp.m21_off[type].push_back(pl.off21 + (type == 0 ? 0 : e2));
            pr.out_off12 = (type == 1 && mode.apply) ? e2 : 0;
            pr.out_off21 = (type == 1 && mode.apply) ? e1 : 0;
            if (type == 1) {
                const long long bound = (long long)a.surf_norm2_max * (long long)b.surf_norm2_max;
                pr.force_exact = bound > 32767LL * 32767LL ? 1 : 0;
            }
            pl.prob_index[type] = (int)bp.probs[type].size();
            bp.mark_off[type].push_back(bp.keep_bytes); bp.keep_bytes += round_up(pr.n1, 16);
            bp.mark_off[type].push_back(bp.keep_bytes); bp.keep_bytes += round_up(pr.n2, 16);
            bp.max_n[type] = std::max(bp.max_n[type], std::max(pr.n1, pr.n2));
            bp.total_queries += pr.n1 + pr.n2;
            bp.probs[type].push_back(pr);
            if (!empty) {
                const int dim = type == 0 ? 128 : 64;
                bp.macs += (int64_t)pr.n1 * pr.n2 * dim;
                if (type == 1) bp.macs_surf += (int64_t)pr.n1 * pr.n2 * dim;
                bp.alg_bytes += (int64_t)(pr.n1 + pr.n2) * (dim + 4);
            }
        }
    }
    bp.bucketed = bp.rs_buckets > 0 && bp.rs_buckets <= INT_MAX && bp.max_n[0] < (1 << 26) && !knobs.rescan_wave;

    std::stable_sort(spentries.begin(), spentries.end(), [](const SpEntry &x, const SpEntry &y) {
        return x.view != y.view ? x.view < y.view : x.units < y.units;
    });
    for (size_t e = 0; e < spentries.size();) {
        SpecialJob j;
        memset(&j, 0, sizeof(j));
        const SpEntry &f = spentries[e];
        if (f.units > kSpSlots) {
            j.problem[0] = f.problem; j.side[0] = f.side; j.count = 0;
            for (int c = 0; c < f.nchunk; ++c) { j.chunk = c; bp.spjobs_wide.push_back(j); }
            ++e;
            continue;
        }
        if (f.units > 1) {
            j.problem[0] = f.problem; j.side[0] = f.side; j.count = 0;
            ++e;
        } else {
            int c = 0;
            while (c < kSpSlots && e < spentries.size() && spentries[e].view == f.view && spentries[e].units == 1) {
                j.problem[c] = spentries[e].problem; j.side[c] = spentries[e].side; ++c; ++e;
            }
            j.count = c;
        }
        for (int c = 0; c < f.nchunk; ++c) { j.chunk = c; bp.spjobs.push_back(j); }
    }
    return OSFM_OK;
}

int batch_size_for(const std::vector<ViewData> &views, const osfm_match_options &o, bool lowres)
{
    if (o.pairs_per_batch > 0) return o.pairs_per_batch;
    if (lowres) return 16384;
    size_t worst = 1;
    for (const auto &v : views) {
        const size_t n = (size_t)std::max(v.ns, v.nu) + 256;
        worst = std::max(worst, (n / kRowsPerBlock + 1) * n * sizeof(ColPart) + n * 64);
    }
    const size_t budget = (size_t)24 << 30;
    return (int)std::max<size_t>(1, std::min<size_t>(budget / worst, 4096));
}

int full_batch_size(const std::vector<ViewData> &views, const osfm_match_options &o, size_t n_full)
{
    int bs = batch_size_for(views, o, false);
    if (o.pairs_per_batch <= 0 && !o.geometric_verification && o.matcher_type != OSFM_MATCHER_CASCADE_HASHING && n_full >= 768)
        bs = std::min<int>(bs, (int)((n_full + 2) / 3));
    if (o.pairs_per_batch <= 0 && n_full > (size_t)bs) {
        const size_t parts = (n_full + bs - 1) / bs;
        bs = (int)((n_full + parts - 1) / parts);
    }
    return bs;
}

void deal_pairs_lpt(const std::vector<ViewData> &views, int num_shards, const osfm_pair *pairs, const std::vector<int> &cand,
    std::vector<std::vector<int>> *owner)
{
    const int n = num_shards;
    owner->assign(n, {});
    const int nc = (int)cand.size();
    std::vector<int64_t> w(nc);
    bool uniform = true;
    for (int i = 0; i < nc; ++i) {
        const ViewData &a = views[pairs[cand[i]].view_1], &b = views[pairs[cand[i]].view_2];
        w[i] = (int64_t)(a.ns + a.nu) * (int64_t)(b.ns + b.nu);
        uniform &= w[i] == w[0];
    }
    if (uniform) {
        for (int i = 0; i < nc; ++i) (*owner)[i % n].push_back(cand[i]);
        return;
    }
    std::vector<int> order(nc);
    for (int i = 0; i < nc; ++i) order[i] = i;
    std::stable_sort(order.begin(), order.end(), [&](int x, int y) { return w[x] > w[y]; });
    typedef std::pair<int64_t, int> Load;
    std::priority_queue<Load, std::vector<Load>, std::greater<Load>> heap;
    for (int k = 0; k < n; ++k) heap.push({0, k});
    std::vector<int> own(nc);
    for (int i : order) {
        Load l = heap.top(); heap.pop();
        own[i] = l.second;
        heap.push({l.first + w[i], l.second});
    }
    for (int i = 0; i < nc; ++i) (*owner)[own[i]].push_back(cand[i]);
}

void build_lowe_table(float lowe, bool is_signed, std::vector<int32_t> *tab)
{
    const volatile float sq = lowe * lowe;
    const float sq_lowe = sq;
    const int dmax = is_signed ? 32258 : 65534;
    tab->assign(32768, 0x7fffffff);
    for (int d2 = 0; d2 <= dmax; d2 += 2) {
        int lo = 0, hi = dmax / 2 + 1;
        while (lo < hi) {
            const int mid = (lo + hi) / 2;
            const float ratio = static_cast<float>(2 * mid) / static_cast<float>(d2);
            if (ratio > sq_lowe) hi = mid; else lo = mid + 1;
        }
        (*tab)[d2 / 2] = lo > dmax / 2 ? 0x7fffffff : 2 * lo;
    }
}

int max_d1_for(float dist_thres, bool is_signed)
{
    const volatile float sq = dist_thres * dist_thres;
    const float sq_dist = sq;
    const int dmax = is_signed ? 32258 : 65534;
    int best = -1;
    int lo = 0, hi = dmax;
    if (!(static_cast<float>(0) > sq_dist)) {
        while (lo < hi) {
            const int mid = (lo + hi + 1) / 2;
            if (static_cast<float>(mid) > sq_dist) hi = mid - 1; else lo = mid;
        }
        best = lo;
    }
    return best;
}

}
```

Baseline: 24020 pairs/s.

## Pipeline full-match chunks across two batch slots with post-processing on copy stream

Splits per-batch device state into two slots and restructures the full matching pass so chunk c+2's tile kernels are enqueued while chunk c is collected, compacted and copied back on a separate post stream. Plans for every chunk are built up front, and buffers are reserved once, sized for the largest chunk. Host staging of compaction lists moves into pinned per-slot memory, so host-to-device uploads can run asynchronously. The design aims to hide host-side decide/compact work and device-to-host list copies behind matching kernels. In exchange it uses more device memory for two slots and adds event and stream complexity.

New measurement: 24260 pairs/s (median of 6 runs). Within noise of the previous version (+1.0%).

```diff
diff --git a/orthosfm_amd/csrc/match_all.hip b/orthosfm_amd/csrc/match_all.hip
--- a/orthosfm_amd/csrc/match_all.hip
+++ b/orthosfm_amd/csrc/match_all.hip
@@ -55,6 +55,117 @@
         OSFM_HIP_CHECK(hipEventRecord(m->ev_copied[cb], m->copy_stream));
         m->copied_used[cb] = true;
     }
+    return OSFM_OK;
+}
+
+int compact_chunk_post(osfm_matcher *m, int slot, const ChunkLists &h, int n, int64_t chunk_corr, int32_t *corr,
+    int64_t written, int chunk_no)
+{
+    hipStream_t post = m->copy_stream;
+    char *hb = m->slot[slot].h_compact;
+    const size_t o_corr = (size_t)n * 8, o_len = (size_t)n * 16, o_keep = (size_t)n * 20;
+    memcpy(hb, h.m12_off.data(), (size_t)n * 8);
+    memcpy(hb + o_corr, h.corr_off.data(), (size_t)n * 8);
+    memcpy(hb + o_len, h.len12.data(), (size_t)n * 4);
+    memcpy(hb + o_keep, h.keep.data(), (size_t)n);
+    DeviceBuffer &dcorr = (chunk_no & 1) ? m->d_corr_alt : m->d_corr;
+    if ((size_t)chunk_corr * 8 > dcorr.bytes) { set_error("match_all: a chunk's lists outgrew their reserve"); return OSFM_E_STATE; }
+    OSFM_HIP_CHECK(hipMemcpyAsync(m->d_m12_off.ptr, hb, (size_t)n * 8, hipMemcpyHostToDevice, post));
+    OSFM_HIP_CHECK(hipMemcpyAsync(m->d_corr_off.ptr, hb + o_corr, (size_t)n * 8, hipMemcpyHostToDevice, post));
+    OSFM_HIP_CHECK(hipMemcpyAsync(m->d_len12.ptr, hb + o_len, (size_t)n * 4, hipMemcpyHostToDevice, post));
+    OSFM_HIP_CHECK(hipMemcpyAsync(m->d_keep_pair.ptr, hb + o_keep, (size_t)n, hipMemcpyHostToDevice, post));
+    launch_compact_pairs(n, m->out.as<int32_t>(), m->d_m12_off.as<int64_t>(),
+        m->d_len12.as<int32_t>(), m->d_corr_off.as<int64_t>(), m->d_keep_pair.as<uint8_t>(),
+        dcorr.as<int32_t>(), post);
+    OSFM_HIP_CHECK(hipGetLastError());
+    OSFM_HIP_CHECK(hipMemcpyAsync(corr + 2 * written, dcorr.ptr, (size_t)chunk_corr * 8, hipMemcpyDeviceToHost, post));
+    return OSFM_OK;
+}
+
+int64_t decide_chunk(const std::vector<int> &full_idx, size_t start, int n, const std::vector<int32_t> &counts,
+    const std::vector<PairPlan> &plans, int min_matches, int64_t written, osfm_pair_result *results, ChunkLists *lists)
+{
+    ChunkLists &h = *lists;
+    h.m12_off.assign(n, 0); h.corr_off.assign(n, 0); h.len12.assign(n, 0); h.keep.assign(n, 0);
+    int64_t chunk_corr = 0;
+    for (int k = 0; k < n; ++k) {
+        const int p = full_idx[start + k];
+        osfm_pair_result &r = results[p];
+        r.num_matches = counts[k];
+        if (counts[k] < min_matches) { r.status = OSFM_PAIR_REJECTED_COUNT; continue; }
+        r.status = OSFM_PAIR_MATCHED;
+        r.offset = written + chunk_corr;
+        h.keep[k] = 1;
+        h.m12_off[k] = plans[k].off12;
+        h.len12[k] = plans[k].len12;
+        h.corr_off[k] = chunk_corr;
+        chunk_corr += counts[k];
+    }
+    return chunk_corr;
+}
+
+int pipelined_pass(osfm_matcher *m, const osfm_pair *pairs, const std::vector<int> &full_idx, int bs, int min_matches,
+    osfm_pair_result *results, int32_t *corr, int64_t capacity, int64_t *written_io, bool *overflow)
+{
+    const osfm_match_options &o = m->opts;
+    const int nchunks = (int)((full_idx.size() + bs - 1) / bs);
+    if (nchunks == 0) return OSFM_OK;
+    hipStream_t post = m->copy_stream;
+    BatchMode full_mode;
+    if (m->expect_pairs > 0)
+        full_mode.expect = std::min<int>(full_batch_size(m->views, o, (size_t)m->expect_pairs), m->expect_pairs);
+
+    if ((int)m->pass_plans.size() < nchunks) m->pass_plans.resize(nchunks);
+    const PlanKnobs knobs = read_plan_knobs();
+    BatchNeeds needs;
+    size_t corr_bytes = 8;
+    std::vector<osfm_pair> chunk;
+    for (int c = 0; c < nchunks; ++c) {
+        const size_t start = (size_t)c * bs, end = std::min(full_idx.size(), start + bs);
+        chunk.clear();
+        for (size_t k = start; k < end; ++k) chunk.push_back(pairs[full_idx[k]]);
+        const int n = (int)chunk.size();
+        BatchPlan &plan = m->pass_plans[c];
+        OSFM_RETURN_IF(plan_batch(m->views, o, m->special_max, knobs, chunk.data(), n, full_mode, &plan));
+        double grow = 1.0;
+        if (full_mode.expect > n && n > 0) grow = 1.02 * (double)full_mode.expect / n;
+        batch_needs(plan, grow, &needs);
+        size_t rows = 0;
+        for (const PairPlan &pl : plan.plans) rows += (size_t)pl.len12;
+        corr_bytes = std::max(corr_bytes, rows * 8);
+    }
+    for (int s = 0; s < std::min(nchunks, 2); ++s) {
+        OSFM_RETURN_IF(reserve_batch(m, s, needs));
+        OSFM_RETURN_IF((s ? m->d_corr_alt : m->d_corr).reserve(corr_bytes));
+    }
+    const size_t nmax = needs.pairs;
+    OSFM_RETURN_IF(m->d_m12_off.reserve(nmax * 8));
+    OSFM_RETURN_IF(m->d_corr_off.reserve(nmax * 8));
+    OSFM_RETURN_IF(m->d_len12.reserve(nmax * 4));
+    OSFM_RETURN_IF(m->d_keep_pair.reserve(nmax));
+
+    OSFM_RETURN_IF(enqueue_tiles(m, 0, &m->pass_plans[0], full_mode));
+    OSFM_RETURN_IF(enqueue_post(m, 0, post));
+    if (nchunks > 1) OSFM_RETURN_IF(enqueue_tiles(m, 1, &m->pass_plans[1], full_mode));
+    int64_t written = *written_io;
+    ChunkLists h;
+    BatchResult res;
+    for (int c = 0; c < nchunks; ++c) {
+        const size_t start = (size_t)c * bs;
+        const BatchPlan &plan = m->pass_plans[c];
+        const int n = (int)plan.plans.size();
+        const Lap lap{};
+        OSFM_RETURN_IF(collect_batch(m, c & 1, &res));
+        lap("collected");
+        const int64_t chunk_corr = decide_chunk(full_idx, start, n, res.counts, plan.plans, min_matches, written, results, &h);
+        if (written + chunk_corr > capacity) *overflow = true;
+        if (chunk_corr > 0 && !*overflow)
+            OSFM_RETURN_IF(compact_chunk_post(m, c & 1, h, n, chunk_corr, corr, written, c));
+        if (c + 1 < nchunks) OSFM_RETURN_IF(enqueue_post(m, (c + 1) & 1, post));
+        if (c + 2 < nchunks) OSFM_RETURN_IF(enqueue_tiles(m, c & 1, &m->pass_plans[c + 2], full_mode));
+        written += chunk_corr;
+    }
+    *written_io = written;
     return OSFM_OK;
 }
 
@@ -149,7 +260,10 @@
     OSFM_HIP_CHECK(hipSetDevice(m->device));
     if (phase != kPhaseFull) reset_stats(m);
     const osfm_match_options &o = m->opts;
-    struct CopyDrain { hipStream_t s; ~CopyDrain() { if (s) (void)hipStreamSynchronize(s); } } copy_drain{m->copy_stream};
+    struct CopyDrain {
+        hipStream_t s[2];
+        ~CopyDrain() { for (hipStream_t x : s) if (x) (void)hipStreamSynchronize(x); }
+    } copy_drain{{m->stream, m->copy_stream}};
 
     std::vector<int> lowres_idx, full_idx;
     for (int p = 0; p < num_pairs; ++p) {
@@ -195,8 +309,13 @@
     const int min_matches = std::max(8, o.min_feature_matches);
     int64_t written = 0, written_out = 0;
     bool overflow = false;
-    {
-        const int bs = full_batch_size(m->views, o, full_idx.size());
+    const char *pipe_env = getenv("OSFM_MATCH_PIPELINE"), *parts_env = getenv("OSFM_PASS_PARTS");
+    const bool pipelined = !(pipe_env && strcmp(pipe_env, "0") == 0) && !o.geometric_verification &&
+        o.matcher_type != OSFM_MATCHER_CASCADE_HASHING;
+    const int bs = full_batch_size(m->views, o, full_idx.size(), parts_env ? atoi(parts_env) : 0);
+    if (pipelined) {
+        OSFM_RETURN_IF(pipelined_pass(m, pairs, full_idx, bs, min_matches, results, corr, capacity, &written, &overflow));
+    } else {
         int chunk_no = 0;
         std::vector<osfm_pair> chunk;
         ChunkLists h;
@@ -212,21 +331,7 @@
                 full_mode.expect = std::min<int>(full_batch_size(m->views, o, (size_t)m->expect_pairs), m->expect_pairs);
             OSFM_RETURN_IF(run_batch(m, chunk.data(), n, full_mode, &res));
             lap("matched");
-            h.m12_off.assign(n, 0); h.corr_off.assign(n, 0); h.len12.assign(n, 0); h.keep.assign(n, 0);
-            int64_t chunk_corr = 0;
-            for (int k = 0; k < n; ++k) {
-                const int p = full_idx[start + k];
-                osfm_pair_result &r = results[p];
-                r.num_matches = res.counts[k];
-                if (res.counts[k] < min_matches) { r.status = OSFM_PAIR_REJECTED_COUNT; continue; }
-                r.status = OSFM_PAIR_MATCHED;
-                r.offset = written + chunk_corr;
-                h.keep[k] = 1;
-                h.m12_off[k] = res.plans[k].off12;
-                h.len12[k] = res.plans[k].len12;
-                h.corr_off[k] = chunk_corr;
-                chunk_corr += res.counts[k];
-            }
+            const int64_t chunk_corr = decide_chunk(full_idx, start, n, res.counts, res.plans, min_matches, written, results, &h);
             if (!o.geometric_verification && written + chunk_corr > capacity) overflow = true;
             if (chunk_corr > 0 && (o.geometric_verification || !overflow))
                 OSFM_RETURN_IF(compact_chunk(m, h, n, chunk_corr, corr, written, &chunk_no));
diff --git a/orthosfm_amd/csrc/match_api.hip b/orthosfm_amd/csrc/match_api.hip
--- a/orthosfm_amd/csrc/match_api.hip
+++ b/orthosfm_amd/csrc/match_api.hip
@@ -147,11 +147,26 @@
     m->views = std::vector<ViewData>(num_views);
     reset_stats(m);
     OSFM_HIP_CHECK(stream_create(&m->stream));
-    for (int i = 0; i < 2; ++i)
-        for (int j = 0; j < 2; ++j) OSFM_HIP_CHECK(event_create(&m->ev[i][j], true));
-    for (int j = 0; j < 2; ++j) OSFM_HIP_CHECK(event_create(&m->ev_sp[j], true));
+    for (osfm::BatchSlot &S : m->slot) {
+        for (int i = 0; i < 2; ++i)
+            for (int j = 0; j < 2; ++j) OSFM_HIP_CHECK(event_create(&S.ev[i][j], true));
+        for (int j = 0; j < 2; ++j) OSFM_HIP_CHECK(event_create(&S.ev_sp[j], true));
+        OSFM_HIP_CHECK(event_create(&S.tiles_done, false));
+        OSFM_HIP_CHECK(event_create(&S.post_done, false));
+    }
     for (int j = 0; j < 2; ++j) OSFM_HIP_CHECK(event_create(&m->pin_ev[j], false));
-    OSFM_HIP_CHECK(stream_create(&m->copy_stream));
+    {
+        const char *prio_env = getenv("OSFM_POST_PRIORITY");
+        int least = 0, greatest = 0;
+        if (prio_env && hipDeviceGetStreamPriorityRange(&least, &greatest) == hipSuccess &&
+            (strcmp(prio_env, "high") == 0 || strcmp(prio_env, "low") == 0)) {
+            OSFM_HIP_CHECK(hipStreamCreateWithPriority(&m->copy_stream, hipStreamNonBlocking,
+                strcmp(prio_env, "high") == 0 ? greatest : least));
+            g_ledger.live_streams++;
+        } else {
+            OSFM_HIP_CHECK(stream_create(&m->copy_stream));
+        }
+    }
     OSFM_HIP_CHECK(stream_create(&m->up_stream));
     for (int j = 0; j < 2; ++j) {
         OSFM_HIP_CHECK(event_create(&m->ev_compact[j], false));
@@ -222,9 +237,14 @@
     }
     (void)hipSetDevice(m->device);
     if (m->stream) (void)hipStreamSynchronize(m->stream);
-    for (int i = 0; i < 2; ++i)
-        for (int j = 0; j < 2; ++j) event_destroy(m->ev[i][j]);
-    for (int j = 0; j < 2; ++j) event_destroy(m->ev_sp[j]);
+    if (m->copy_stream) (void)hipStreamSynchronize(m->copy_stream);
+    for (osfm::BatchSlot &S : m->slot) {
+        for (int i = 0; i < 2; ++i)
+            for (int j = 0; j < 2; ++j) event_destroy(S.ev[i][j]);
+        for (int j = 0; j < 2; ++j) event_destroy(S.ev_sp[j]);
+        event_destroy(S.tiles_done);
+        event_destroy(S.post_done);
+    }
     for (int j = 0; j < 2; ++j) {
         event_destroy(m->pin_ev[j]);
         pinned_free(m->pin_ptr[j], m->pin_bytes[j]);
diff --git a/orthosfm_amd/csrc/match_batch.hip b/orthosfm_amd/csrc/match_batch.hip
--- a/orthosfm_amd/csrc/match_batch.hip
+++ b/orthosfm_amd/csrc/match_batch.hip
@@ -11,179 +11,279 @@
 
 void reset_stats(osfm_matcher *m) { memset(&m->stats, 0, sizeof(m->stats)); }
 
-int run_batch(osfm_matcher *m, const osfm_pair *pairs, int num_pairs, const BatchMode &mode,
-    BatchResult *res)
-{
-    const bool cascade = cascade_batch(m->opts, mode);
-    if (cascade) OSFM_RETURN_IF(ensure_cashash(m));
+PlanKnobs read_plan_knobs()
+{
     static const int forced_seg_tiles = [] { const char *e = getenv("OSFM_SEG_TILES"); return e ? atoi(e) : 0; }();
     const char *rescan_env = getenv("OSFM_FINISH_RESCAN");
     PlanKnobs knobs;
     knobs.seg_tiles = forced_seg_tiles;
     knobs.rescan_wave = rescan_env && strcmp(rescan_env, "wave") == 0;
-    BatchPlan &plan = m->plan;
-    res->counts.assign(num_pairs, 0);
-    OSFM_RETURN_IF(plan_batch(m->views, m->opts, m->special_max, knobs, pairs, num_pairs, mode, &plan));
-    res->plans = plan.plans;
-    res->out_ints = plan.out_ints;
-    const std::vector<PairPlan> &plans = plan.plans;
-    std::vector<MatchProblem> *probs = plan.probs;
-    const std::vector<SpecialJob> &spjobs = plan.spjobs, &spjobs_wide = plan.spjobs_wide;
-    const int64_t out_ints = plan.out_ints, total_queries = plan.total_queries, rs_buckets = plan.rs_buckets;
-    const int *total_blocks = plan.total_blocks, *max_n = plan.max_n;
-
-    double grow = 1.0;
-    if (mode.expect > num_pairs && num_pairs > 0) grow = 1.02 * (double)mode.expect / num_pairs;
+    return knobs;
+}
+
+namespace {
+
+BatchSlot::PinLayout pin_layout(const size_t np[2], size_t nsp, size_t pairs)
+{
+    BatchSlot::PinLayout l;
+    size_t at = 0;
+    auto take = [&](size_t bytes) { const size_t here = at; at += (bytes + 255) / 256 * 256; return here; };
+    for (int type = 0; type < 2; ++type) l.probs[type] = take(np[type] * sizeof(MatchProblem));
+    for (int type = 0; type < 2; ++type) l.mark[type] = take(np[type] * 2 * sizeof(int64_t));
+    l.spjobs = take(nsp * sizeof(SpecialJob));
+    for (int type = 0; type < 2; ++type) l.counts[type] = take(np[type] * sizeof(int32_t));
+    l.exact = take(16);
+    l.probe = take(16);
+    l.compact = take(pairs * 21);
+    l.total = at;
+    return l;
+}
+
+}
+
+void batch_needs(const BatchPlan &plan, double grow, BatchNeeds *needs)
+{
     auto grown = [&](int64_t n) { return (size_t)((double)std::max<int64_t>(n, 1) * std::max(grow, 1.0)); };
-    OSFM_RETURN_IF(m->out.reserve(grown(std::max<int64_t>(out_ints, 4)) * 4));
-    OSFM_RETURN_IF(m->rowparts.reserve(grown(plan.rowpart_recs) * sizeof(RowPart)));
-    OSFM_RETURN_IF(m->colparts.reserve(grown(plan.colpart_recs) * sizeof(ColPart)));
-    OSFM_RETURN_IF(m->keep.reserve(grown(std::max<int64_t>(plan.keep_bytes, 16))));
-    OSFM_RETURN_IF(m->exact_items.reserve(grown(total_queries) * sizeof(ExactItem)));
-    OSFM_RETURN_IF(m->exact_count.reserve(16));
+    auto up = [](size_t &to, size_t v) { to = std::max(to, v); };
+    up(needs->out, grown(std::max<int64_t>(plan.out_ints, 4)) * 4);
+    up(needs->rowparts, grown(plan.rowpart_recs) * sizeof(RowPart));
+    up(needs->colparts, grown(plan.colpart_recs) * sizeof(ColPart));
+    up(needs->keep, grown(std::max<int64_t>(plan.keep_bytes, 16)));
+    up(needs->exact_items, grown(plan.total_queries) * sizeof(ExactItem));
     if (plan.bucketed) {
-        OSFM_RETURN_IF(m->rs_count.reserve(grown(rs_buckets) * sizeof(int32_t)));
-        OSFM_RETURN_IF(m->rs_items.reserve(grown(plan.rs_items) * sizeof(RescoreItem)));
-    }
-    OSFM_RETURN_IF(m->sp_parts.reserve((size_t)std::max<int64_t>(plan.sp_recs, 1) * sizeof(RowPart)));
+        up(needs->rs_count, grown(plan.rs_buckets) * sizeof(int32_t));
+        up(needs->rs_items, grown(plan.rs_items) * sizeof(RescoreItem));
+    }
+    up(needs->sp_parts, (size_t)std::max<int64_t>(plan.sp_recs, 1) * sizeof(RowPart));
+    up(needs->sp_col, (size_t)std::max<int64_t>(plan.sp_cols, 1) * 4);
+    up(needs->d_spjobs, std::max<size_t>(plan.spjobs.size() + plan.spjobs_wide.size(), 1) * sizeof(SpecialJob));
+    for (int type = 0; type < 2; ++type) {
+        up(needs->problems[type], plan.probs[type].size());
+        if (plan.cascade && !plan.probs[type].empty())
+            up(needs->cas_state, (size_t)std::max<int64_t>(plan.cas_queries[type], 1) * kCasMaxCand * 4);
+    }
+    up(needs->pairs, plan.plans.size());
+}
+
+int reserve_batch(osfm_matcher *m, int slot, const BatchNeeds &n)
+{
+    BatchSlot &S = m->slot[slot];
+    OSFM_RETURN_IF(m->out.reserve(n.out));
+    OSFM_RETURN_IF(S.rowparts.reserve(n.rowparts));
+    OSFM_RETURN_IF(S.colparts.reserve(n.colparts));
+    OSFM_RETURN_IF(m->keep.reserve(n.keep));
+    OSFM_RETURN_IF(m->exact_items.reserve(n.exact_items));
+    OSFM_RETURN_IF(S.exact_count.reserve(16));
+    OSFM_RETURN_IF(S.clock_probe.reserve(16));
+    OSFM_RETURN_IF(m->rs_count.reserve(n.rs_count));
+    OSFM_RETURN_IF(m->rs_items.reserve(n.rs_items));
+    OSFM_RETURN_IF(m->sp_parts.reserve(n.sp_parts));
+    OSFM_RETURN_IF(m->sp_col.reserve(n.sp_col));
+    OSFM_RETURN_IF(m->d_spjobs.reserve(n.d_spjobs));
+    OSFM_RETURN_IF(m->cas_state.reserve(n.cas_state));
+    for (int type = 0; type < 2; ++type) {
+        OSFM_RETURN_IF(S.d_problems[type].reserve(n.problems[type] * sizeof(MatchProblem)));
+        OSFM_RETURN_IF(S.mark_off[type].reserve(n.problems[type] * 2 * sizeof(int64_t)));
+        OSFM_RETURN_IF(S.counts[type].reserve(n.problems[type] * sizeof(int32_t)));
+    }
+    S.lay_problems[0] = n.problems[0]; S.lay_problems[1] = n.problems[1];
+    S.lay_spjobs = n.d_spjobs / sizeof(SpecialJob); S.lay_pairs = n.pairs;
+    S.lay = pin_layout(S.lay_problems, S.lay_spjobs, S.lay_pairs);
+    OSFM_RETURN_IF(S.pin.reserve(S.lay.total));
+    if (!m->zero_tile.ptr) {
+        OSFM_RETURN_IF(m->zero_tile.reserve((size_t)kTileCols * 128));
+        OSFM_HIP_CHECK(hipMemsetAsync(m->zero_tile.ptr, 0, (size_t)kTileCols * 128, m->stream));
+    }
+    return OSFM_OK;
+}
+
+int enqueue_tiles(osfm_matcher *m, int slot, BatchPlan *plan, const BatchMode &mode)
+{
+    BatchSlot &S = m->slot[slot];
+    S.plan = plan; S.mode = mode;
+    S.timed[0] = S.timed[1] = S.probed = false;
+    const bool cascade = plan->cascade;
+    std::vector<MatchProblem> *probs = plan->probs;
+    const BatchSlot::PinLayout &lay = S.lay;
+    if (probs[0].size() > S.lay_problems[0] || probs[1].size() > S.lay_problems[1] || plan->plans.size() > S.lay_pairs ||
+        plan->spjobs.size() + plan->spjobs_wide.size() > S.lay_spjobs || lay.total > S.pin.bytes) {
+        set_error("match: a batch was queued without its reserve");
+        return OSFM_E_STATE;
+    }
+    S.special = !cascade && !(plan->spjobs.empty() && plan->spjobs_wide.empty());
+    for (int type = 0; type < 2; ++type) S.h_counts[type] = reinterpret_cast<int32_t *>(S.pin.ptr + lay.counts[type]);
+    S.h_exact = reinterpret_cast<int32_t *>(S.pin.ptr + lay.exact);
+    S.h_probe = reinterpret_cast<unsigned long long *>(S.pin.ptr + lay.probe);
+    S.h_compact = S.pin.ptr + lay.compact;
     hipStream_t s = m->stream;
+    OSFM_HIP_CHECK(hipStreamWaitEvent(s, S.post_done, 0));
     {
         std::vector<uint8_t> seen(m->views.size(), 0);
-        for (int p = 0; p < num_pairs; ++p)
-            for (int v : {plans[p].v1, plans[p].v2})
+        for (const PairPlan &pl : plan->plans)
+            for (int v : {pl.v1, pl.v2})
                 if (!seen[v]) { seen[v] = 1; if (m->views[v].ready) OSFM_HIP_CHECK(hipStreamWaitEvent(s, m->views[v].ready, 0)); }
     }
-    OSFM_RETURN_IF(m->sp_col.reserve((size_t)std::max<int64_t>(plan.sp_cols, 1) * 4));
-    OSFM_RETURN_IF(m->d_spjobs.reserve(std::max<size_t>(spjobs.size() + spjobs_wide.size(), 1) * sizeof(SpecialJob)));
-    if (!spjobs.empty())
-        OSFM_HIP_CHECK(hipMemcpyAsync(m->d_spjobs.ptr, spjobs.data(), spjobs.size() * sizeof(SpecialJob),
-            hipMemcpyHostToDevice, s));
-    if (!spjobs_wide.empty())
-        OSFM_HIP_CHECK(hipMemcpyAsync(m->d_spjobs.as<SpecialJob>() + spjobs.size(), spjobs_wide.data(),
-            spjobs_wide.size() * sizeof(SpecialJob), hipMemcpyHostToDevice, s));
     int32_t *d_out = m->out.as<int32_t>();
-    OSFM_HIP_CHECK(hipMemsetAsync(d_out, 0xff, (size_t)std::max<int64_t>(out_ints, 4) * 4, s));
-
-    OSFM_HIP_CHECK(hipMemsetAsync(m->exact_count.ptr, 0, 16, s));
-    bool timed[2] = {false, false};
-    bool probed = false;
+    if (cascade) OSFM_HIP_CHECK(hipMemsetAsync(d_out, 0xff, (size_t)std::max<int64_t>(plan->out_ints, 4) * 4, s));
     for (int type = 0; type < 2; ++type) {
         const int np = (int)probs[type].size();
         if (np == 0) continue;
         for (int i = 0; i < np; ++i) {
-            probs[type][i].m12 = d_out + plan.m12_off[type][i];
-            probs[type][i].m21 = d_out + plan.m21_off[type][i];
+            probs[type][i].m12 = d_out + plan->m12_off[type][i];
+            probs[type][i].m21 = d_out + plan->m21_off[type][i];
         }
-        OSFM_RETURN_IF(m->d_problems[type].reserve(np * sizeof(MatchProblem)));
-        OSFM_RETURN_IF(m->mark_off[type].reserve(np * 2 * sizeof(int64_t)));
-        OSFM_RETURN_IF(m->counts[type].reserve(np * sizeof(int32_t)));
-        OSFM_HIP_CHECK(hipMemcpyAsync(m->d_problems[type].ptr, probs[type].data(),
+        memcpy(S.pin.ptr + lay.probs[type], probs[type].data(), np * sizeof(MatchProblem));
+        OSFM_HIP_CHECK(hipMemcpyAsync(S.d_problems[type].ptr, S.pin.ptr + lay.probs[type],
             np * sizeof(MatchProblem), hipMemcpyHostToDevice, s));
-        OSFM_HIP_CHECK(hipMemcpyAsync(m->mark_off[type].ptr, plan.mark_off[type].data(),
-            np * 2 * sizeof(int64_t), hipMemcpyHostToDevice, s));
-        OSFM_HIP_CHECK(hipMemsetAsync(m->counts[type].ptr, 0, np * sizeof(int32_t), s));
-        const MatchProblem *dp = m->d_problems[type].as<MatchProblem>();
+        const MatchProblem *dp = S.d_problems[type].as<MatchProblem>();
+        const LoweTable tab = type == 0 ? m->tab_sift : m->tab_surf;
+        if (cascade) {
+            OSFM_HIP_CHECK(hipEventRecord(S.ev[type][0], s));
+            S.timed[type] = true;
+            launch_cashash_match(type == 0 ? 128 : 64, dp, np, plan->max_n[type], m->cas_state.as<int32_t>(), tab, s);
+            OSFM_HIP_CHECK(hipEventRecord(S.ev[type][1], s));
+        } else {
+            if (plan->total_blocks[type] > 0) { OSFM_HIP_CHECK(hipEventRecord(S.ev[type][0], s)); S.timed[type] = true; }
+            unsigned long long *probe = nullptr;
+            if (type == 0 && mode.limit == 0) {
+                OSFM_HIP_CHECK(hipMemsetAsync(S.clock_probe.ptr, 0, 16, s));
+                probe = S.clock_probe.as<unsigned long long>();
+                S.probed = true;
+            }
+            launch_match_tiles(type == 0 ? 8 : 4, plan->needs_mask[type], plan->any_special[type], plan->any_c0[type],
+                plan->any_corrected[type], dp, np, plan->total_blocks[type],
+                S.rowparts.as<RowPart>(), S.colparts.as<ColPart>(), s, probe, m->zero_tile.as<int8_t>());
+            if (S.timed[type]) OSFM_HIP_CHECK(hipEventRecord(S.ev[type][1], s));
+        }
+        OSFM_HIP_CHECK(hipGetLastError());
+    }
+    OSFM_HIP_CHECK(hipEventRecord(S.tiles_done, s));
+    return OSFM_OK;
+}
+
+int enqueue_post(osfm_matcher *m, int slot, hipStream_t post)
+{
+    BatchSlot &S = m->slot[slot];
+    const BatchPlan &plan = *S.plan;
+    const BatchMode &mode = S.mode;
+    const std::vector<SpecialJob> &spjobs = plan.spjobs, &spjobs_wide = plan.spjobs_wide;
+    const size_t np2[2] = {plan.probs[0].size(), plan.probs[1].size()};
+    const BatchSlot::PinLayout &lay = S.lay;
+    const int64_t total_queries = plan.total_queries, rs_buckets = plan.rs_buckets;
+    if (S.special) {
+        SpecialJob *h = reinterpret_cast<SpecialJob *>(S.pin.ptr + lay.spjobs);
+        if (!spjobs.empty()) memcpy(h, spjobs.data(), spjobs.size() * sizeof(SpecialJob));
+        if (!spjobs_wide.empty()) memcpy(h + spjobs.size(), spjobs_wide.data(), spjobs_wide.size() * sizeof(SpecialJob));
+        OSFM_HIP_CHECK(hipMemcpyAsync(m->d_spjobs.ptr, h, (spjobs.size() + spjobs_wide.size()) * sizeof(SpecialJob),
+            hipMemcpyHostToDevice, post));
+    }
+    if (!plan.cascade)
+        OSFM_HIP_CHECK(hipMemsetAsync(m->out.ptr, 0xff, (size_t)std::max<int64_t>(plan.out_ints, 4) * 4, post));
+    OSFM_HIP_CHECK(hipMemsetAsync(S.exact_count.ptr, 0, 16, post));
+    for (int type = 0; type < 2; ++type) {
+        const size_t np = np2[type];
+        if (np == 0) continue;
+        memcpy(S.pin.ptr + lay.mark[type], plan.mark_off[type].data(), np * 2 * sizeof(int64_t));
+        OSFM_HIP_CHECK(hipMemcpyAsync(S.mark_off[type].ptr, S.pin.ptr + lay.mark[type], np * 2 * sizeof(int64_t),
+            hipMemcpyHostToDevice, post));
+        OSFM_HIP_CHECK(hipMemsetAsync(S.counts[type].ptr, 0, np * sizeof(int32_t), post));
+    }
+    const bool rs = !plan.cascade && np2[0] > 0 && plan.bucketed;
+    if (rs) OSFM_HIP_CHECK(hipMemsetAsync(m->rs_count.ptr, 0, (size_t)rs_buckets * sizeof(int32_t), post));
+    if (post != m->stream) OSFM_HIP_CHECK(hipStreamWaitEvent(post, S.tiles_done, 0));
+    for (int type = 0; type < 2; ++type) {
+        const int np = (int)np2[type];
+        if (np == 0) continue;
+        const MatchProblem *dp = S.d_problems[type].as<MatchProblem>();
         const LoweTable tab = type == 0 ? m->tab_sift : m->tab_surf;
         const int ecap = (int)std::min<int64_t>(total_queries, 0x7fffffff);
-        int32_t *ecount = m->exact_count.as<int32_t>() + type;
-
-        if (cascade) {
-            OSFM_HIP_CHECK(hipEventRecord(m->ev[type][0], s));
-            timed[type] = true;
-            OSFM_RETURN_IF(m->cas_state.reserve((size_t)std::max<int64_t>(plan.cas_queries[type], 1) * kCasMaxCand * 4));
-            launch_cashash_match(type == 0 ? 128 : 64, dp, np, max_n[type], m->cas_state.as<int32_t>(), tab, s);
-            OSFM_HIP_CHECK(hipEventRecord(m->ev[type][1], s));
-        } else {
-            if (total_blocks[type] > 0) { OSFM_HIP_CHECK(hipEventRecord(m->ev[type][0], s)); timed[type] = true; }
-            unsigned long long *probe = nullptr;
-            if (type == 0 && mode.limit == 0) {
-                OSFM_RETURN_IF(m->clock_probe.reserve(16));
-                OSFM_HIP_CHECK(hipMemsetAsync(m->clock_probe.ptr, 0, 16, s));
-                probe = m->clock_probe.as<unsigned long long>();
-                probed = true;
+        int32_t *ecount = S.exact_count.as<int32_t>() + type;
+        if (!plan.cascade) {
+            if (type == 0 && S.special) {
+                OSFM_HIP_CHECK(hipEventRecord(S.ev_sp[0], post));
+                launch_match_special(dp, m->d_spjobs.as<SpecialJob>(), (int)spjobs.size(), m->sp_parts.as<RowPart>(),
+                    m->sp_col.as<int32_t>(), post);
+                launch_match_special_wide(dp, m->d_spjobs.as<SpecialJob>() + spjobs.size(), (int)spjobs_wide.size(),
+                    m->sp_parts.as<RowPart>(), m->sp_col.as<int32_t>(), post);
+                OSFM_HIP_CHECK(hipEventRecord(S.ev_sp[1], post));
             }
-            if (!m->zero_tile.ptr) {
-                OSFM_RETURN_IF(m->zero_tile.reserve((size_t)kTileCols * 128));
-                OSFM_HIP_CHECK(hipMemsetAsync(m->zero_tile.ptr, 0, (size_t)kTileCols * 128, s));
-            }
-            launch_match_tiles(type == 0 ? 8 : 4, plan.needs_mask[type], plan.any_special[type], plan.any_c0[type],
-                plan.any_corrected[type], dp, np, total_blocks[type],
-                m->rowparts.as<RowPart>(), m->colparts.as<ColPart>(), s, probe, m->zero_tile.as<int8_t>());
-            if (timed[type]) OSFM_HIP_CHECK(hipEventRecord(m->ev[type][1], s));
-            if (type == 0 && !(spjobs.empty() && spjobs_wide.empty())) {
-                OSFM_HIP_CHECK(hipEventRecord(m->ev_sp[0], s));
-                launch_match_special(dp, m->d_spjobs.as<SpecialJob>(), (int)spjobs.size(), m->sp_parts.as<RowPart>(),
-                    m->sp_col.as<int32_t>(), s);
-                launch_match_special_wide(dp, m->d_spjobs.as<SpecialJob>() + spjobs.size(), (int)spjobs_wide.size(),
-                    m->sp_parts.as<RowPart>(), m->sp_col.as<int32_t>(), s);
-                OSFM_HIP_CHECK(hipEventRecord(m->ev_sp[1], s));
-            }
-            const bool rs = type == 0 && plan.bucketed;
-            if (rs) OSFM_HIP_CHECK(hipMemsetAsync(m->rs_count.ptr, 0, (size_t)rs_buckets * sizeof(int32_t), s));
-            launch_match_finish(dp, np, max_n[type], m->rowparts.as<RowPart>(),
-                m->colparts.as<ColPart>(), m->sp_parts.as<RowPart>(), m->sp_col.as<int32_t>(), tab, 0,
-                m->exact_items.as<ExactItem>(), ecount, ecap, rs ? m->rs_count.as<int32_t>() : nullptr,
-                rs ? m->rs_items.as<RescoreItem>() : nullptr, s);
-            if (rs)
+            const bool rs_type = rs && type == 0;
+            launch_match_finish(dp, np, plan.max_n[type], S.rowparts.as<RowPart>(),
+                S.colparts.as<ColPart>(), m->sp_parts.as<RowPart>(), m->sp_col.as<int32_t>(), tab, 0,
+                m->exact_items.as<ExactItem>(), ecount, ecap, rs_type ? m->rs_count.as<int32_t>() : nullptr,
+                rs_type ? m->rs_items.as<RescoreItem>() : nullptr, post);
+            if (rs_type)
                 launch_match_rescore(dp, np, m->rs_count.as<int32_t>(), m->rs_items.as<RescoreItem>(), rs_buckets, tab,
-                    m->exact_items.as<ExactItem>(), ecount, ecap, s);
+                    m->exact_items.as<ExactItem>(), ecount, ecap, post);
             launch_exact_scan(type == 0 ? 128 : 64, dp, m->exact_items.as<ExactItem>(), ecount, ecap,
-                tab, s);
+                tab, post);
         }
-        launch_cross_check_mark(dp, np, max_n[type], m->keep.as<uint8_t>(), m->keep.as<uint8_t>(),
-            m->mark_off[type].as<int64_t>(), m->counts[type].as<int32_t>(), s);
+        launch_cross_check_mark(dp, np, plan.max_n[type], m->keep.as<uint8_t>(), m->keep.as<uint8_t>(),
+            S.mark_off[type].as<int64_t>(), S.counts[type].as<int32_t>(), post);
         if (mode.apply)
-            launch_cross_check_apply(dp, np, max_n[type], m->keep.as<uint8_t>(),
-                m->keep.as<uint8_t>(), m->mark_off[type].as<int64_t>(), s);
+            launch_cross_check_apply(dp, np, plan.max_n[type], m->keep.as<uint8_t>(),
+                m->keep.as<uint8_t>(), S.mark_off[type].as<int64_t>(), post);
         OSFM_HIP_CHECK(hipGetLastError());
     }
 
-    std::vector<int32_t> hc[2];
-    int32_t hexact[4] = {0, 0, 0, 0};
-    for (int type = 0; type < 2; ++type) {
-        hc[type].resize(probs[type].size());
-        if (!hc[type].empty())
-            OSFM_HIP_CHECK(hipMemcpyAsync(hc[type].data(), m->counts[type].ptr,
-                hc[type].size() * sizeof(int32_t), hipMemcpyDeviceToHost, s));
-    }
-    OSFM_HIP_CHECK(hipMemcpyAsync(hexact, m->exact_count.ptr, 16, hipMemcpyDeviceToHost, s));
-    unsigned long long hprobe[2] = {0, 0};
-    if (probed) OSFM_HIP_CHECK(hipMemcpyAsync(hprobe, m->clock_probe.ptr, 16, hipMemcpyDeviceToHost, s));
-    OSFM_HIP_CHECK(hipStreamSynchronize(s));
-    m->stats.tile_shader_cycles += (double)hprobe[0];
-    m->stats.tile_refclk_ticks += (double)hprobe[1];
-    for (int p = 0; p < num_pairs; ++p) {
+    for (int type = 0; type < 2; ++type)
+        if (np2[type] > 0)
+            OSFM_HIP_CHECK(hipMemcpyAsync(S.h_counts[type], S.counts[type].ptr, np2[type] * sizeof(int32_t),
+                hipMemcpyDeviceToHost, post));
+    OSFM_HIP_CHECK(hipMemcpyAsync(S.h_exact, S.exact_count.ptr, 16, hipMemcpyDeviceToHost, post));
+    S.h_probe[0] = S.h_probe[1] = 0;
+    if (S.probed) OSFM_HIP_CHECK(hipMemcpyAsync(S.h_probe, S.clock_probe.ptr, 16, hipMemcpyDeviceToHost, post));
+    OSFM_HIP_CHECK(hipEventRecord(S.post_done, post));
+    return OSFM_OK;
+}
+
+int enqueue_batch(osfm_matcher *m, int slot, BatchPlan *plan, const BatchMode &mode)
+{
+    OSFM_RETURN_IF(enqueue_tiles(m, slot, plan, mode));
+    return enqueue_post(m, slot, m->stream);
+}
+
+int collect_batch(osfm_matcher *m, int slot, BatchResult *res)
+{
+    BatchSlot &S = m->slot[slot];
+    const BatchPlan &plan = *S.plan;
+    const std::vector<PairPlan> &plans = plan.plans;
+    OSFM_HIP_CHECK(hipEventSynchronize(S.post_done));
+    m->stats.tile_shader_cycles += (double)S.h_probe[0];
+    m->stats.tile_refclk_ticks += (double)S.h_probe[1];
+    res->counts.assign(plans.size(), 0);
+    for (size_t p = 0; p < plans.size(); ++p) {
         int c = 0;
         for (int type = 0; type < 2; ++type)
-            if (plans[p].prob_index[type] >= 0) c += hc[type][plans[p].prob_index[type]];
+            if (plans[p].prob_index[type] >= 0) c += S.h_counts[type][plans[p].prob_index[type]];
         res->counts[p] = c;
     }
     for (int type = 0; type < 2; ++type) {
-        if (!timed[type]) continue;
+        if (!S.timed[type]) continue;
         float ms = 0.f;
-        OSFM_HIP_CHECK(hipEventElapsedTime(&ms, m->ev[type][0], m->ev[type][1]));
-        if (cascade) {
+        OSFM_HIP_CHECK(hipEventElapsedTime(&ms, S.ev[type][0], S.ev[type][1]));
+        if (plan.cascade) {
             m->stats.cashash_kernel_ms += ms;
             m->stats.cashash_kernel_launches += 1;
-        } else if (mode.limit > 0) {
+        } else if (S.mode.limit > 0) {
             m->stats.lowres_kernel_ms += ms;
             m->stats.lowres_kernel_launches += 1;
         } else {
             m->stats.tile_kernel_ms += ms;
             m->stats.tile_kernel_launches += 1;
-            m->stats.tile_workgroups += total_blocks[type];
+            m->stats.tile_workgroups += plan.total_blocks[type];
             if (type == 1) { m->stats.surf_tile_kernel_ms += ms; m->stats.surf_tile_kernel_launches += 1; }
         }
     }
-    if (!(spjobs.empty() && spjobs_wide.empty())) {
+    if (S.special) {
         float ms = 0.f;
-        OSFM_HIP_CHECK(hipEventElapsedTime(&ms, m->ev_sp[0], m->ev_sp[1]));
+        OSFM_HIP_CHECK(hipEventElapsedTime(&ms, S.ev_sp[0], S.ev_sp[1]));
         m->stats.special_kernel_ms += ms;
         m->stats.special_kernel_launches += 1;
     }
-    m->stats.exact_scan_queries += hexact[0] + hexact[1];
-    if (cascade) {
-    } else if (mode.limit > 0) {
+    m->stats.exact_scan_queries += S.h_exact[0] + S.h_exact[1];
+    if (plan.cascade) {
+    } else if (S.mode.limit > 0) {
         m->stats.lowres_mac_count += plan.macs;
     } else {
         m->stats.mac_count += plan.macs;
@@ -193,4 +293,22 @@
     return OSFM_OK;
 }
 
-}
+int run_batch(osfm_matcher *m, const osfm_pair *pairs, int num_pairs, const BatchMode &mode,
+    BatchResult *res)
+{
+    if (cascade_batch(m->opts, mode)) OSFM_RETURN_IF(ensure_cashash(m));
+    BatchPlan &plan = m->plan;
+    res->counts.assign(num_pairs, 0);
+    OSFM_RETURN_IF(plan_batch(m->views, m->opts, m->special_max, read_plan_knobs(), pairs, num_pairs, mode, &plan));
+    res->plans = plan.plans;
+    res->out_ints = plan.out_ints;
+    double grow = 1.0;
+    if (mode.expect > num_pairs && num_pairs > 0) grow = 1.02 * (double)mode.expect / num_pairs;
+    BatchNeeds needs;
+    batch_needs(plan, grow, &needs);
+    OSFM_RETURN_IF(reserve_batch(m, 0, needs));
+    OSFM_RETURN_IF(enqueue_batch(m, 0, &plan, mode));
+    return collect_batch(m, 0, res);
+}
+
+}
diff --git a/orthosfm_amd/csrc/match_internal.h b/orthosfm_amd/csrc/match_internal.h
--- a/orthosfm_amd/csrc/match_internal.h
+++ b/orthosfm_amd/csrc/match_internal.h
@@ -8,6 +8,55 @@
 #include <vector>
 
 #include "match_plan.h"
+
+namespace osfm {
+
+struct PinnedBlock {
+    char *ptr = nullptr;
+    size_t bytes = 0;
+    PinnedBlock() = default;
+    PinnedBlock(const PinnedBlock &) = delete;
+    PinnedBlock &operator=(const PinnedBlock &) = delete;
+    ~PinnedBlock() { pinned_free(ptr, bytes); }
+    int reserve(size_t need)
+    {
+        if (need <= bytes) return OSFM_OK;
+        pinned_free(ptr, bytes);
+        ptr = nullptr; bytes = 0;
+        const size_t want = need + need / 4 + 256;
+        OSFM_HIP_CHECK(pinned_alloc(reinterpret_cast<void **>(&ptr), want, hipHostMallocDefault));
+        bytes = want;
+        return OSFM_OK;
+    }
+};
+
+struct BatchSlot {
+    DeviceBuffer d_problems[2];
+    DeviceBuffer rowparts, colparts;
+    DeviceBuffer clock_probe;
+    DeviceBuffer mark_off[2], counts[2], exact_count;
+    hipEvent_t ev[2][2] = {{nullptr, nullptr}, {nullptr, nullptr}};
+    hipEvent_t ev_sp[2] = {nullptr, nullptr};
+    hipEvent_t tiles_done = nullptr, post_done = nullptr;
+    PinnedBlock pin;
+    struct PinLayout { size_t probs[2], mark[2], spjobs, counts[2], exact, probe, compact, total; } lay = {};
+    size_t lay_problems[2] = {0, 0}, lay_spjobs = 0, lay_pairs = 0;
+    const BatchPlan *plan = nullptr;
+    BatchMode mode;
+    bool timed[2] = {false, false}, probed = false, special = false;
+    int32_t *h_counts[2] = {nullptr, nullptr}, *h_exact = nullptr;
+    unsigned long long *h_probe = nullptr;
+    char *h_compact = nullptr;
+};
+
+struct BatchNeeds {
+    size_t out = 0, rowparts = 0, colparts = 0, keep = 0, exact_items = 0, rs_count = 0, rs_items = 0;
+    size_t sp_parts = 0, sp_col = 0, d_spjobs = 0, cas_state = 0;
+    size_t problems[2] = {0, 0};
+    size_t pairs = 0;
+};
+
+}
 
 struct osfm_matcher {
     int device = 0;
@@ -20,12 +69,13 @@
     hipStream_t up_stream = nullptr;
     std::mutex up_mu;
 
-    osfm::DeviceBuffer d_problems[2], rowparts, colparts, out, keep, mark_off[2], counts[2];
-    osfm::DeviceBuffer exact_items, exact_count, stage_in, flags;
+    osfm::BatchSlot slot[2];
+    osfm::DeviceBuffer out, keep;
+    osfm::DeviceBuffer exact_items, stage_in, flags;
     osfm::DeviceBuffer rs_count, rs_items;
     osfm::DeviceBuffer sp_parts, sp_col, d_spjobs;
-    osfm::DeviceBuffer clock_probe;
     osfm::BatchPlan plan;
+    std::vector<osfm::BatchPlan> pass_plans;
     osfm::DeviceBuffer zero_tile;
     int special_max = 512;
     int expect_pairs = 0;
@@ -35,8 +85,6 @@
     hipEvent_t ev_compact[2] = {nullptr, nullptr}, ev_copied[2] = {nullptr, nullptr};
     bool copied_used[2] = {false, false};
     osfm::DeviceBuffer d_jobs, d_inl, d_inl_count, d_corr2, d_gather_off;
-    hipEvent_t ev[2][2] = {{nullptr, nullptr}, {nullptr, nullptr}};
-    hipEvent_t ev_sp[2] = {nullptr, nullptr};
     char *pin_ptr[2] = {nullptr, nullptr};
     size_t pin_bytes[2] = {0, 0};
     hipEvent_t pin_ev[2] = {nullptr, nullptr};
@@ -76,6 +124,13 @@
 
 int check_view(const osfm_matcher *m, int v, const char *what);
 int run_batch(osfm_matcher *m, const osfm_pair *pairs, int num_pairs, const BatchMode &mode, BatchResult *res);
+PlanKnobs read_plan_knobs();
+void batch_needs(const BatchPlan &plan, double grow, BatchNeeds *needs);
+int reserve_batch(osfm_matcher *m, int slot, const BatchNeeds &needs);
+int enqueue_tiles(osfm_matcher *m, int slot, BatchPlan *plan, const BatchMode &mode);
+int enqueue_post(osfm_matcher *m, int slot, hipStream_t post);
+int enqueue_batch(osfm_matcher *m, int slot, BatchPlan *plan, const BatchMode &mode);
+int collect_batch(osfm_matcher *m, int slot, BatchResult *res);
 void reset_stats(osfm_matcher *m);
 
 int upload_view(osfm_matcher *m, int view, const uint16_t *sift, int n_sift, const int16_t *surf, int n_surf);
diff --git a/orthosfm_amd/csrc/match_plan.h b/orthosfm_amd/csrc/match_plan.h
--- a/orthosfm_amd/csrc/match_plan.h
+++ b/orthosfm_amd/csrc/match_plan.h
@@ -85,7 +85,8 @@
     const osfm_pair *pairs, int num_pairs, const BatchMode &mode, BatchPlan *out);
 
 int batch_size_for(const std::vector<ViewData> &views, const osfm_match_options &o, bool lowres);
-int full_batch_size(const std::vector<ViewData> &views, const osfm_match_options &o, size_t n_full);
+constexpr int kPassParts = 3;
+int full_batch_size(const std::vector<ViewData> &views, const osfm_match_options &o, size_t n_full, int parts = 0);
 
 void deal_pairs_lpt(const std::vector<ViewData> &views, int num_shards, const osfm_pair *pairs, const std::vector<int> &cand,
     std::vector<std::vector<int>> *owner);
diff --git a/orthosfm_amd/csrc/match_plan.hip b/orthosfm_amd/csrc/match_plan.hip
--- a/orthosfm_amd/csrc/match_plan.hip
+++ b/orthosfm_amd/csrc/match_plan.hip
@@ -232,11 +232,12 @@
     return (int)std::max<size_t>(1, std::min<size_t>(budget / worst, 4096));
 }
 
-int full_batch_size(const std::vector<ViewData> &views, const osfm_match_options &o, size_t n_full)
+int full_batch_size(const std::vector<ViewData> &views, const osfm_match_options &o, size_t n_full, int parts_wanted)
 {
     int bs = batch_size_for(views, o, false);
+    const size_t cut = parts_wanted > 0 ? parts_wanted : kPassParts;
     if (o.pairs_per_batch <= 0 && !o.geometric_verification && o.matcher_type != OSFM_MATCHER_CASCADE_HASHING && n_full >= 768)
-        bs = std::min<int>(bs, (int)((n_full + 2) / 3));
+        bs = std::min<int>(bs, (int)((n_full + cut - 1) / cut));
     if (o.pairs_per_batch <= 0 && n_full > (size_t)bs) {
         const size_t parts = (n_full + bs - 1) / bs;
         bs = (int)((n_full + parts - 1) / parts);
```
